# brownvc/matryodshka

Measured on AMD Instinct MI355X. Metric: novel-view frames/sec, 640x320 ODS->32-sphere MSI infer+render, higher is better.
Workload: dtype f32

## Files before the change

### matryodshka_amd/csrc/cnn_device.h

```cpp
#pragma once
#include <cmath>
#include <cstdint>
#include <cstdio>
#include <cstdlib>
#include <cstring>
#include <new>
#include <type_traits>
#include <vector>

#include "msi_common.h"

namespace msi_cnn {


typedef float f32x16 __attribute__((ext_vector_type(16)));
typedef float v4f __attribute__((ext_vector_type(4)));
typedef __attribute__((address_space(3))) void lds_void;

constexpr int BK = 32;
constexpr int ROW_BYTES = BK * 4;
#ifndef MSI_NSTAGE
#define MSI_NSTAGE 2
#endif
constexpr int NSTAGE = MSI_NSTAGE;
constexpr int NPAD_ALIGN = 128;
constexpr int COORD_CLASSES = 5;
[[maybe_unused]] constexpr unsigned OOB = 0x80000000u;
constexpr int DEFAULT_CUS = 256;
constexpr int MAX_SPLIT = 8;
constexpr int CONV_SLOTS_PER_CU = 5;
constexpr double LN_EPS = 1e-12;
constexpr int LN_SHARDS = 64, LN_WORDS = 2;
constexpr int LN_S1_BITS = 24, LN_S2_BITS = 16;
constexpr int LN_SCL_DOUBLES = 4;
constexpr double LN_UNDERFLOW_UNITS_SQ = 1e12;
enum { STATUS_APPLY_AHEAD_TIMEOUT = 1, STATUS_LN_OVERFLOW = 2, STATUS_LN_UNDERFLOW = 4, STATUS_F16_SPLIT_RANGE = 8 };
constexpr int AP_FLAG_STRIDE = 16;
constexpr int HEAD_MAX_C = 256;

enum { MODE_CONV = 0, MODE_CONVT = 1, MODE_HEAD = 2 };

struct ConvParams {
  const char *x0, *x1;
  const char *wpk;
  const char *wpk_x3;
  const float *coord_bias;
  int cb_stride;
  const double *ln_scl;
  const double *ln_scl_src, *ln_scl_src1;
  int *status;
  const long long *ln_sums;
  const float *ln_gamma, *ln_beta;
  double ln_inv_n;
  const long long *ln_sums1;
  const float *ln_gamma1, *ln_beta1;
  double ln_inv_n1;
  int halo_apply;
  const float *bias;
  float *y;
  long long *sums;
  float *partial;
  int *tile_cnt;
  int tiles_m, tiles_n, ntiles;
  int n_main, split0, split;
  int nb_main;
  int C0, C1;
  int Hin, Win, Hout, Wout, Cout, npad;
  int Mh, Mw;
  unsigned mg_mw, mg_tm, mg_tn, mg_nc, mg_sp0, mg_sp;
  int ntaps, cpt0, cpt1, ksteps;
  int stride, rate, pad_t, pad_l;
  int mode, wrap, nclass;
  int halo_tx;
  unsigned mg_htx;
  int halo_xor;
  int row_par;
  float *ap_x;
  unsigned short *ap_yb;
  const long long *ap_sums;
  const float *ap_gamma, *ap_beta;
  float *ap_aff;
  int *ap_flags;
  int *ap_err;
  double ap_inv_n;
  int n_apply, ap_units_per_row, ap_unit_vec, ap_row_vec;
#if defined(MSI_CONV_TIMING) || defined(MSI_DEBUG_STATS)
  unsigned long long *dbg;
#endif
};

enum ConvFamily {
  CONV_IGEMM = 0,
  CONV_HALO, CONV_HALO_S2, CONVT_HALO,
  CONV_HALO_X3, CONV_HALO8_X3, CONV_HALO_S2_X3, CONV_HALO8_S2_X3, CONVT_HALO_X3, CONVT_HALO8_X3,
  CONV_HALO_BF16, CONV_HALO_BF16_S2, CONVT_HALO_BF16,
};
struct ConvVariant {
  int family;
  int bm, bn;
  int mode, bf16;
  int rate;
  int apply;
  int planes;
  int waves;
  bool is_halo() const { return family != CONV_IGEMM; }
  bool is_convt_f32() const { return family == CONVT_HALO || family == CONVT_HALO_X3 || family == CONVT_HALO8_X3; }
  bool is_convt() const { return is_convt_f32() || family == CONVT_HALO_BF16; }
  bool six_product() const { return family >= CONV_HALO_X3 && family <= CONVT_HALO8_X3; }
  bool tile8() const { return family == CONV_HALO8_X3 || family == CONV_HALO8_S2_X3 || family == CONVT_HALO8_X3; }
};

struct LayerLaunch {
  ConvParams p;
  ConvVariant variant;
  int nblocks, nfix;
  int inlaunch;
  int fuse_ln;
  int skip_apply;
  unsigned ln_blocks;
};

constexpr int HA_TP = 32;
#ifndef MSI_HA_LG
#define MSI_HA_LG 32
#endif
constexpr int HA_LG = MSI_HA_LG;

struct HeadAsmParams {
  const float *x;
  const float *wpk;
  const float *bias;
  const float *aff;
  const void *psv;
  float4 *rgba;
  float *bw_out, *al_out;
  float *pred_out;
  int C0, ksteps, npad, nd, hw;
  int lg, ng;
  unsigned mg_vpp, mg_nchunk, mg_hw;
  long npix_total;
  void *layers;
};

int launch_conv(const LayerLaunch &Q, const ConvParams &p, hipStream_t stream);
int launch_igemm(const LayerLaunch &Q, const ConvParams &p, hipStream_t stream);
int launch_fixup(int bm, int bn, int mode, int raw16, unsigned grid_x, unsigned grid_y, const ConvParams &p, hipStream_t stream);
int launch_halo_f32(const LayerLaunch &Q, const ConvParams &p, hipStream_t stream);
int launch_x3(const LayerLaunch &Q, const ConvParams &p, hipStream_t stream);
int launch_bf16_halo(const LayerLaunch &Q, const ConvParams &p, hipStream_t stream);
int launch_zero(void *p, size_t n16, hipStream_t stream);
int launch_ln_finish(int batch, hipStream_t stream, const long long *sums, double inv_n, const double *scl, int *status, const float *gamma, const float *beta, int C,
                     float *aff, int raw16);
int launch_ln_apply(int bf16out, unsigned blocks, int batch, size_t lds, hipStream_t stream, float *x, const long long *sums, double inv_n, const double *scl, int *status,
                    const float *gamma, const float *beta, size_t per_sample, int C, float *aff, unsigned short *yb);
int launch_head_assemble(int bf16in, int format, unsigned grid_x, size_t lds, hipStream_t stream, const HeadAsmParams &q);
int debug_conv_occupancy(int lds_bytes);

constexpr int vkey(int family, int a = 0, int b = 0, int c = 0, int d = 0, int e = 0) { return ((((family * 16 + a) * 16 + b) * 16 + c) * 16 + d) * 16 + e; }

inline int set_max_lds(const void *fn, int lds, unsigned long long &done, const char *what) {
  int dev = 0;
  if (hipGetDevice(&dev) != hipSuccess) dev = 0;
  const bool tracked = dev >= 0 && dev < 64;
  if (tracked && ((done >> dev) & 1ull)) return MSI_OK;
  hipError_t e = hipFuncSetAttribute(fn, hipFuncAttributeMaxDynamicSharedMemorySize, lds);
  if (e != hipSuccess) return msi::fail(MSI_E_LAUNCH, "%s: %s", what, hipGetErrorString(e));
  if (tracked) done |= 1ull << dev;
  return MSI_OK;
}

template <auto KERNEL, int LDS, int THREADS = 256>
int launch_kernel(unsigned nblocks, const ConvParams &p, hipStream_t stream, const char *what) {
  if constexpr (LDS > 65536) {
    static thread_local unsigned long long done = 0;
    int rc0 = set_max_lds(reinterpret_cast<const void *>(KERNEL), LDS, done, what);
    if (rc0) return rc0;
  }
  hipLaunchKernelGGL(KERNEL, dim3(nblocks), dim3(THREADS), LDS, stream, p);
  return msi::check_launch(what);
}

template <int N> using IC = std::integral_constant<int, N>;
}
using namespace msi_cnn;

namespace {

template <int MODE>
__device__ __forceinline__ int tap_delta(int v, int parity, int rate, bool wrapt) {
  if (MODE == MODE_CONV) return v * rate;
  if (MODE == MODE_CONVT) return wrapt ? -v : (v == 0 ? 0 : (parity ? 1 : -1));
  return 0;
}

__device__ __forceinline__ unsigned udiv_magic(unsigned x, unsigned d, unsigned mg) {
  unsigned q = __umulhi(x, mg);
  if (x - q * d >= d) ++q;
  return q;
}

__device__ __forceinline__ int halo_row(const ConvParams &p, int tyi, int r, int rows_per_tile) {
  return p.row_par ? (tyi >> 1) * (2 * rows_per_tile) + (tyi & 1) + 2 * r : tyi * rows_per_tile + r;
}

__device__ __forceinline__ float msi_tanh(float x) {
  const float xa = fminf(fabsf(x), 15.0f);
  const float t = __builtin_amdgcn_exp2f(xa * 2.8853900817779268f);
  const float r = (t - 1.0f) * __builtin_amdgcn_rcpf(t + 1.0f);
  return x != x ? x : __builtin_copysignf(r, x);
}

__device__ __forceinline__ int coord_class(int mw, int Mw) {
  return mw < 2 ? mw : (mw >= Mw - 2 ? 3 + (mw - (Mw - 2)) : 2);
}

template <int N>
__device__ __forceinline__ void wait_vmcnt() {
  asm volatile("s_waitcnt vmcnt(%0)" ::"n"(N) : "memory");
}

template <int OFF>
__device__ __forceinline__ v4f lds_read128(unsigned addr) {
  v4f v;
  if constexpr (OFF < 65536) {
    asm volatile("ds_read_b128 %0, %1 offset:%2" : "=v"(v) : "v"(addr), "n"(OFF) : "memory");
  } else {
    asm volatile("ds_read_b128 %0, %1 offset:%2" : "=v"(v) : "v"(addr + (OFF & ~0xffff)), "n"(OFF & 0xffff) : "memory");
  }
  return v;
}
template <int N>
__device__ __forceinline__ void wait_lgkm(v4f &x, v4f &y) {
  asm volatile("s_waitcnt lgkmcnt(%2)" : "+v"(x), "+v"(y) : "n"(N) : "memory");
}
template <int N, int MT, int NT>
__device__ __forceinline__ void wait_lgkm_frag(v4f (&a)[MT], v4f (&b)[NT]) {
  static_assert((MT == 1 || MT == 2 || MT == 4) && (NT == 1 || NT == 2), "fragment shapes of the conv kernels");
  if constexpr (MT == 1 && NT == 1) asm volatile("s_waitcnt lgkmcnt(%2)" : "+v"(a[0]), "+v"(b[0]) : "n"(N) : "memory");
  else if constexpr (MT == 2 && NT == 1) asm volatile("s_waitcnt lgkmcnt(%3)" : "+v"(a[0]), "+v"(a[1]), "+v"(b[0]) : "n"(N) : "memory");
  else if constexpr (MT == 1 && NT == 2) asm volatile("s_waitcnt lgkmcnt(%3)" : "+v"(a[0]), "+v"(b[0]), "+v"(b[1]) : "n"(N) : "memory");
  else if constexpr (MT == 2 && NT == 2) asm volatile("s_waitcnt lgkmcnt(%4)" : "+v"(a[0]), "+v"(a[1]), "+v"(b[0]), "+v"(b[1]) : "n"(N) : "memory");
  else if constexpr (MT == 4 && NT == 1) asm volatile("s_waitcnt lgkmcnt(%5)" : "+v"(a[0]), "+v"(a[1]), "+v"(a[2]), "+v"(a[3]), "+v"(b[0]) : "n"(N) : "memory");
  else asm volatile("s_waitcnt lgkmcnt(%6)" : "+v"(a[0]), "+v"(a[1]), "+v"(a[2]), "+v"(a[3]), "+v"(b[0]), "+v"(b[1]) : "n"(N) : "memory");
}

__device__ __forceinline__ float wave_sum(float x) {
#define MSI_DPP_ADD(CTRL, ROWMASK)                                                                                     \
  x += __builtin_bit_cast(float, __builtin_amdgcn_update_dpp(0, __builtin_bit_cast(int, x), CTRL, ROWMASK, 0xf, true))
  MSI_DPP_ADD(0xB1, 0xf);
  MSI_DPP_ADD(0x4E, 0xf);
  MSI_DPP_ADD(0x141, 0xf);
  MSI_DPP_ADD(0x140, 0xf);
  MSI_DPP_ADD(0x142, 0xa);
  MSI_DPP_ADD(0x143, 0xc);
#undef MSI_DPP_ADD
  return __builtin_bit_cast(float, __builtin_amdgcn_readlane(__builtin_bit_cast(int, x), 63));
}

__device__ __forceinline__ double wave_sum_f64(double x) {
#define MSI_DPP_ADD64(CTRL, ROWMASK)                                                                                   \
  {                                                                                                                    \
    const long long b_ = __builtin_bit_cast(long long, x);                                                             \
    const int lo_ = __builtin_amdgcn_update_dpp(0, (int)b_, CTRL, ROWMASK, 0xf, true);                                 \
    const int hi_ = __builtin_amdgcn_update_dpp(0, (int)(b_ >> 32), CTRL, ROWMASK, 0xf, true);                         \
    x += __builtin_bit_cast(double, ((long long)hi_ << 32) | (unsigned)lo_);                                           \
  }
  MSI_DPP_ADD64(0xB1, 0xf) MSI_DPP_ADD64(0x4E, 0xf) MSI_DPP_ADD64(0x141, 0xf) MSI_DPP_ADD64(0x140, 0xf)
  MSI_DPP_ADD64(0x142, 0xa) MSI_DPP_ADD64(0x143, 0xc)
#undef MSI_DPP_ADD64
  const long long b = __builtin_bit_cast(long long, x);
  const int lo = __builtin_amdgcn_readlane((int)b, 63), hi = __builtin_amdgcn_readlane((int)(b >> 32), 63);
  return __builtin_bit_cast(double, ((long long)hi << 32) | (unsigned)lo);
}

__device__ __forceinline__ void ln_atomic_add(long long *dst, double x_scaled, int *status) {
  const double MAGIC = 6755399441055744.0;
  if (!(fabs(x_scaled) < 2251799813685248.0 )) {
    if (status) __hip_atomic_fetch_or(status, STATUS_LN_OVERFLOW, __ATOMIC_RELAXED, __HIP_MEMORY_SCOPE_AGENT);
    return;
  }
  const double t = x_scaled + MAGIC;
  const long long v = __builtin_bit_cast(long long, t) - __builtin_bit_cast(long long, MAGIC);
  __hip_atomic_fetch_add(dst, v, __ATOMIC_RELAXED, __HIP_MEMORY_SCOPE_AGENT);
}

struct LnShard { long long w0, w1; };
__device__ __forceinline__ LnShard ln_shard_load(const long long *sums, int tid) {
  LnShard r = {0, 0};
  if (tid < 64) {
    const long long *s = sums + (size_t)tid * LN_WORDS;
    r.w0 = s[0]; r.w1 = s[1];
  }
  return r;
}
template <bool PRE>
__device__ __forceinline__ void ln_mean_inv_impl(const long long *sums, LnShard pre, double inv_n, const double *scl, int *status, double *s_stat, int tid) {
  static_assert(LN_SHARDS == 64, "one shard per lane of wave 0");
  const double inv_s1 = scl[2], inv_s2 = scl[3];
  if (tid < 64) {
    long long w0 = pre.w0, w1 = pre.w1;
    if constexpr (!PRE) {
      const long long *s = sums + (size_t)tid * LN_WORDS;
      w0 = s[0]; w1 = s[1];
    }
    const double h1 = wave_sum_f64((double)w0), h2 = wave_sum_f64((double)w1);
    if (tid == 0) {
      const double S1 = h1 * inv_s1, S2 = h2 * inv_s2;
      if (status && h2 * h2 < LN_UNDERFLOW_UNITS_SQ * (1.0 / (inv_n * 1024.0) + 1.0))
        __hip_atomic_fetch_or(status, STATUS_LN_UNDERFLOW, __ATOMIC_RELAXED, __HIP_MEMORY_SCOPE_AGENT);
      const double mu = S1 * inv_n;
      double var = S2 * inv_n - mu * mu;
      var = var > 0.0 ? var : 0.0;
      const double x = var + LN_EPS, hx = 0.5 * x;
      double r = __builtin_amdgcn_rsq(x);
      r = r * (1.5 - hx * r * r);
      r = r * (1.5 - hx * r * r);
      s_stat[0] = mu;
      s_stat[1] = r;
    }
  }
  __syncthreads();
}
__device__ __forceinline__ void ln_mean_inv(const long long *sums, double inv_n, const double *scl, int *status, double *s_stat, int tid) {
  ln_mean_inv_impl<false>(sums, LnShard{0, 0}, inv_n, scl, status, s_stat, tid);
}
__device__ __forceinline__ void ln_mean_inv_pre(LnShard pre, double inv_n, const double *scl, int *status, double *s_stat, int tid) {
  ln_mean_inv_impl<true>(nullptr, pre, inv_n, scl, status, s_stat, tid);
}

typedef unsigned u32x4_t __attribute__((ext_vector_type(4)));

#ifndef MSI_HANDOFF_FENCE
#define MSI_HANDOFF_FENCE 0
#endif
#ifndef MSI_HANDOFF_AUX
#define MSI_HANDOFF_AUX 16
#endif
__device__ __forceinline__ void handoff_release() {
  if (MSI_HANDOFF_FENCE & 1) __builtin_amdgcn_fence(__ATOMIC_RELEASE, "agent");
}
__device__ __forceinline__ void handoff_acquire() {
  if (MSI_HANDOFF_FENCE & 2) __builtin_amdgcn_fence(__ATOMIC_ACQUIRE, "agent");
}

template <int MT, int NT, int AUX>
__device__ __forceinline__ void dump_acc(const f32x16 (&acc)[MT][NT], __amdgpu_buffer_rsrc_t rsrc, int tid) {
#pragma unroll
  for (int i = 0; i < MT; ++i)
#pragma unroll
    for (int j = 0; j < NT; ++j)
#pragma unroll
      for (int g = 0; g < 4; ++g) {
        const v4f v = {acc[i][j][4 * g], acc[i][j][4 * g + 1], acc[i][j][4 * g + 2], acc[i][j][4 * g + 3]};
        __builtin_amdgcn_raw_buffer_store_b128(__builtin_bit_cast(u32x4_t, v), rsrc,
                                               (unsigned)((((i * NT + j) * 4 + g) * 256 + tid) * 16), 0, AUX);
      }
}

template <int MT, int NT, int AUX>
__device__ __forceinline__ void sum_slabs(f32x16 (&acc)[MT][NT], __amdgpu_buffer_rsrc_t rsrc, int nsp, int slab_bytes, int tid) {
  for (int s = 0; s < nsp; ++s) {
    v4f t[MT][NT][4];
#pragma unroll
    for (int i = 0; i < MT; ++i)
#pragma unroll
      for (int j = 0; j < NT; ++j)
#pragma unroll
        for (int g = 0; g < 4; ++g)
          t[i][j][g] = __builtin_bit_cast(v4f, (u32x4_t)__builtin_amdgcn_raw_buffer_load_b128(
              rsrc, (unsigned)((((i * NT + j) * 4 + g) * 256 + tid) * 16), s * slab_bytes, AUX));
#pragma unroll
    for (int i = 0; i < MT; ++i)
#pragma unroll
      for (int j = 0; j < NT; ++j)
#pragma unroll
        for (int g = 0; g < 4; ++g) {
          if (s == 0) {
            acc[i][j][4 * g] = t[i][j][g].x; acc[i][j][4 * g + 1] = t[i][j][g].y;
            acc[i][j][4 * g + 2] = t[i][j][g].z; acc[i][j][4 * g + 3] = t[i][j][g].w;
          } else {
            acc[i][j][4 * g] += t[i][j][g].x; acc[i][j][4 * g + 1] += t[i][j][g].y;
            acc[i][j][4 * g + 2] += t[i][j][g].z; acc[i][j][4 * g + 3] += t[i][j][g].w;
          }
        }
  }
}

constexpr int EPI_STAGE_BYTES = 48 * 1024;
#ifndef MSI_EPI_NT
#define MSI_EPI_NT 0
#endif
#ifndef MSI_EPI_ABLATE
#define MSI_EPI_ABLATE 0
#endif
#ifdef MSI_CONV_TIMING
#define MSI_STAMP(k) { if (p.dbg && tid == 0) p.dbg[(size_t)blockIdx.x * 24 + (k)] = __builtin_amdgcn_s_memtime(); }
#else
#define MSI_STAMP(k)
#endif
template <int BM, int BN, int MODE, int RAW16, bool CB, bool STAGED, int WR>
__device__ __forceinline__ void emit_whole_tile(const ConvParams &p, f32x16 (&acc)[BM / (32 * WR)][BN / 64], int tile_m, int tile_n, int cls,
                                                int b, int tid, const v4f (&cb_pre)[4], bool use_pre, float pivot, float raw_mul,
                                                double scl_s1, double scl_s2, char *stage) {
  constexpr int MT = BM / (32 * WR), NT = BN / 64, NG = NT * 4, YSZ = RAW16 ? 2 : 4;
  constexpr int ROWB = NT * 32 * YSZ, PITCH = ROWB + 16, NP = ROWB / 16, PPI = 64 / NP, NRD = 32 / PPI;
  constexpr bool FITS = 2 * WR * MT * 32 * PITCH <= EPI_STAGE_BYTES;
  typedef float v2f __attribute__((ext_vector_type(2)));
  typedef _Float16 h2_t __attribute__((ext_vector_type(2)));
  typedef unsigned u2_t __attribute__((ext_vector_type(2)));
  const int lane = tid & 63, wave = tid >> 6, wm = wave >> 1, wn = wave & 1, half = lane >> 5;
  const int ph = cls >> 1, pw = cls & 1;
  const int mtot = p.Mh * p.Mw;
  const bool want_stats = p.sums != nullptr;
  const float pv_s = pivot * raw_mul;
  const v2f rm = {raw_mul, raw_mul}, pv = {pv_s, pv_s};
  const int nbw = tile_n * BN + wn * (NT * 32), nb0 = nbw + 4 * half;
  const size_t sample_bytes = (size_t)(MODE == MODE_CONVT ? p.Hout * p.Wout : mtot) * p.Cout * YSZ;
  constexpr bool staged = STAGED;
  static_assert(!STAGED || FITS, "staging strips");
  const int tyi = p.halo_tx ? (int)udiv_magic((unsigned)tile_m, (unsigned)p.halo_tx, p.mg_htx) : 0;
  const int txi = tile_m - tyi * p.halo_tx;
  MSI_STAMP(16)
  char *yp[MT];
  const float *cbp[MT];
#pragma unroll
  for (int i = 0; i < MT; ++i) {
    yp[i] = nullptr; cbp[i] = nullptr;
    if (CB || !staged) {
      int m = tile_m * BM + wm * (MT * 32) + i * 32 + (lane & 31);
      if (p.halo_tx) {
        const int local = wm * (MT * 32) + i * 32 + (lane & 31);
        m = halo_row(p, tyi, local >> 4, BM / 16) * p.Mw + txi * 16 + ((local & 15) ^ (((local >> 4) & 1) * p.halo_xor));
      }
      int mh = 0, mw = 0;
      if (MODE == MODE_CONVT || CB) {
        mh = (int)udiv_magic((unsigned)m, (unsigned)p.Mw, p.mg_mw);
        mw = m - mh * p.Mw;
      }
      const size_t opix = MODE == MODE_CONVT ? ((size_t)b * p.Hout + (2 * mh + ph)) * p.Wout + (2 * mw + pw) : (size_t)b * mtot + m;
      yp[i] = reinterpret_cast<char *>(p.y) + (opix * p.Cout + nb0) * YSZ;
      if (CB) cbp[i] = p.coord_bias + (size_t)(mh * COORD_CLASSES + coord_class(mw, p.Mw)) * p.cb_stride + nb0;
    }
  }
  char *wst = stage + wave * (MT * 32 * PITCH);
  const int slot = p.halo_tx ? ((lane & 16) | ((lane & 15) ^ (((lane >> 4) & 1) * p.halo_xor))) : (lane & 31);
  char *wp = wst + slot * PITCH + half * (4 * YSZ);
  v2f s1v[4] = {}, s2v[4] = {};
#pragma unroll
  for (int i = 0; i < MT; ++i) {
    v2f ya[NG], yc[NG];
#pragma unroll
    for (int q = 0; q < NG; ++q) {
      ya[q] = v2f{acc[i][q >> 2][4 * (q & 3)], acc[i][q >> 2][4 * (q & 3) + 1]};
      yc[q] = v2f{acc[i][q >> 2][4 * (q & 3) + 2], acc[i][q >> 2][4 * (q & 3) + 3]};
    }
    if (CB) {
      v4f cb[NG];
#pragma unroll
      for (int q = 0; q < NG; ++q)
        cb[q] = (MT == 1 && NT == 1 && use_pre) ? cb_pre[q & 3] : *reinterpret_cast<const v4f *>(cbp[i] + (q >> 2) * 32 + 8 * (q & 3));
#pragma unroll
      for (int q = 0; q < NG; ++q) { ya[q] += v2f{cb[q].x, cb[q].y}; yc[q] += v2f{cb[q].z, cb[q].w}; }
    }
    if (RAW16) {
#pragma unroll
      for (int q = 0; q < NG; ++q) { ya[q] *= rm; yc[q] *= rm; }
    }
    u2_t hw[NG];
    if (RAW16) {
#pragma unroll
      for (int q = 0; q < NG; ++q) {
        const h2_t lo = {(_Float16)ya[q].x, (_Float16)ya[q].y}, hi = {(_Float16)yc[q].x, (_Float16)yc[q].y};
        hw[q] = u2_t{__builtin_bit_cast(unsigned, lo), __builtin_bit_cast(unsigned, hi)};
      }
    }
    if (!(MSI_EPI_ABLATE & 1)) {
#pragma unroll
      for (int q = 0; q < NG; ++q) {
        char *dst = staged ? wp + i * (32 * PITCH) : yp[i];
        if (RAW16) *reinterpret_cast<u2_t *>(dst + ((q >> 2) * 32 + 8 * (q & 3)) * 2) = hw[q];
        else *reinterpret_cast<v4f *>(dst + ((q >> 2) * 32 + 8 * (q & 3)) * 4) = v4f{ya[q].x, ya[q].y, yc[q].x, yc[q].y};
      }
    }
    if (want_stats && !(MSI_EPI_ABLATE & 4)) {
#pragma unroll
      for (int q = 0; q < NG; ++q) { ya[q] -= pv; yc[q] -= pv; }
#pragma unroll
      for (int q = 0; q < NG; ++q) { s1v[q & 3] += ya[q]; s1v[q & 3] += yc[q]; }
#pragma unroll
      for (int q = 0; q < NG; ++q) {
        s2v[q & 3] = __builtin_elementwise_fma(ya[q], ya[q], s2v[q & 3]);
        s2v[q & 3] = __builtin_elementwise_fma(yc[q], yc[q], s2v[q & 3]);
      }
    }
  }
  MSI_STAMP(21)
  const v2f t1 = (s1v[0] + s1v[1]) + (s1v[2] + s1v[3]), t2 = (s2v[0] + s2v[1]) + (s2v[2] + s2v[3]);
  float s1 = t1.x + t1.y, s2 = t2.x + t2.y;
  if (staged && !(MSI_EPI_ABLATE & 1)) {
    const char *rp = wst + (lane / NP) * PITCH + (lane % NP) * 16;
    v4f pc[MT][NRD];
#pragma unroll
    for (int i = 0; i < MT; ++i)
#pragma unroll
      for (int k = 0; k < NRD; ++k) pc[i][k] = *reinterpret_cast<const v4f *>(rp + (i * 32 + k * PPI) * PITCH);
    const __amdgpu_buffer_rsrc_t rsrc_y = __builtin_amdgcn_make_buffer_rsrc(reinterpret_cast<char *>(p.y) + (size_t)b * sample_bytes, 0, (int)(unsigned)sample_bytes, 0x00020000);
    const int rowb = p.Cout * YSZ;
    int pix0, rowstep, colstep;
    if (p.halo_tx) {
      const int r0 = halo_row(p, tyi, wm * (MT * 2), BM / 16), c0 = txi * 16 + lane / NP;
      if (MODE == MODE_CONVT) { pix0 = (2 * r0 + ph) * p.Wout + 2 * c0 + pw; rowstep = 2 * p.Wout; colstep = 2; }
      else { pix0 = r0 * p.Mw + c0; rowstep = p.row_par ? 2 * p.Mw : p.Mw; colstep = 1; }
    } else {
      pix0 = tile_m * BM + wm * (MT * 32) + lane / NP; rowstep = 16; colstep = 1;
    }
    const unsigned v0 = (unsigned)pix0 * (unsigned)rowb + (unsigned)(nbw * YSZ + (lane % NP) * 16);
#pragma unroll
    for (int i = 0; i < MT; ++i)
#pragma unroll
      for (int k = 0; k < NRD; ++k) {
        const int ro = 2 * i + ((k * PPI) >> 4), co = (k * PPI) & 15;
        __builtin_amdgcn_raw_buffer_store_b128(__builtin_bit_cast(u32x4_t, pc[i][k]), rsrc_y, v0 + (unsigned)((ro * rowstep + co * colstep) * rowb), 0, MSI_EPI_NT ? 2 : 0);
      }
  }
  MSI_STAMP(17)
  if (want_stats) {
    s1 = wave_sum(s1); s2 = wave_sum(s2);
    MSI_STAMP(18)
    if (lane == 0 && !(MSI_EPI_ABLATE & 2)) {
      const double P = (double)pv_s, n = (double)(MT * NT * 16 * 64), a = (double)s1;
      const double u1 = RAW16 ? 16777216.0 : scl_s1, u2 = RAW16 ? 65536.0 : scl_s2;
      if (RAW16 && !(s2 <= 1.0727e9f)) __hip_atomic_fetch_or(p.status, STATUS_LN_OVERFLOW, __ATOMIC_RELAXED, __HIP_MEMORY_SCOPE_AGENT);
      long long *dst = p.sums + ((size_t)b * LN_SHARDS + ((blockIdx.x * 4 + wave) & (LN_SHARDS - 1))) * LN_WORDS;
      ln_atomic_add(dst, (n * P + a) * u1, p.status);
      ln_atomic_add(dst + 1, ((double)s2 + 2.0 * P * a + n * P * P) * u2, p.status);
    }
    MSI_STAMP(19)
  }
}

template <int BM, int BN, int MODE, bool INTERIOR, int RAW16, int WR>
__device__ __forceinline__ void emit_tile_impl(const ConvParams &p, f32x16 (&acc)[BM / (32 * WR)][BN / 64], int tile_m,
                                               int tile_n, int cls, int b, int tid, const v4f (&cb_pre)[4], bool use_pre, char *stage,
                                               float raw_mul_pre) {
  constexpr int MT = BM / (32 * WR), NT = BN / 64;
  const int lane = tid & 63, wave = tid >> 6, wm = wave >> 1, wn = wave & 1, half = lane >> 5;
  const int ph = cls >> 1, pw = cls & 1;
  const int mtot = p.Mh * p.Mw;
  const bool wrapt = MODE == MODE_CONVT && p.wrap != 0;
  const bool vec_ok = (p.Cout & 3) == 0;
  const bool has_cb = MODE == MODE_CONV && p.coord_bias != nullptr;
  const bool want_stats = MODE != MODE_HEAD && p.sums != nullptr;
  const float pivot = __builtin_bit_cast(float, __builtin_amdgcn_readfirstlane(__builtin_bit_cast(int, acc[0][0][0])));
  double scl_s1 = 0.0, scl_s2 = 0.0;
  const bool have_pre = INTERIOR && RAW16 && MODE != MODE_HEAD && raw_mul_pre > 0.f;
  if ((want_stats || RAW16) && !have_pre) { scl_s1 = p.ln_scl[0]; scl_s2 = p.ln_scl[1]; }
  const float raw_mul = have_pre ? raw_mul_pre : RAW16 ? (float)(scl_s1 * (1.0 / 16777216.0)) : 1.f;
  constexpr int YSZ = RAW16 ? 2 : 4;
  float s1 = 0.f, s2 = 0.f, cnt = 0.f;
  if constexpr (INTERIOR && MODE != MODE_HEAD) {
    constexpr bool FITS = 2 * WR * MT * 32 * (NT * 32 * (RAW16 ? 2 : 4) + 16) <= EPI_STAGE_BYTES;
    const size_t sample_bytes = (size_t)(MODE == MODE_CONVT ? p.Hout * p.Wout : p.Mh * p.Mw) * p.Cout * (RAW16 ? 2 : 4);
    const bool staged = FITS && stage != nullptr && sample_bytes < 0xfffffff0ull && (p.halo_tx != 0 || MODE == MODE_CONV);
    if constexpr (FITS) {
      if (staged) {
        if (has_cb) emit_whole_tile<BM, BN, MODE, RAW16, true, true, WR>(p, acc, tile_m, tile_n, cls, b, tid, cb_pre, use_pre, pivot, raw_mul, scl_s1, scl_s2, stage);
        else emit_whole_tile<BM, BN, MODE, RAW16, false, true, WR>(p, acc, tile_m, tile_n, cls, b, tid, cb_pre, use_pre, pivot, raw_mul, scl_s1, scl_s2, stage);
        return;
      }
    }
    if (has_cb) emit_whole_tile<BM, BN, MODE, RAW16, true, false, WR>(p, acc, tile_m, tile_n, cls, b, tid, cb_pre, use_pre, pivot, raw_mul, scl_s1, scl_s2, stage);
    else emit_whole_tile<BM, BN, MODE, RAW16, false, false, WR>(p, acc, tile_m, tile_n, cls, b, tid, cb_pre, use_pre, pivot, raw_mul, scl_s1, scl_s2, stage);
    return;
  }
#pragma unroll
  for (int i = 0; i < MT; ++i) {
    int m = tile_m * BM + wm * (MT * 32) + i * 32 + (lane & 31);
    if ((MODE == MODE_CONV || MODE == MODE_CONVT) && p.halo_tx) {
      const int local = wm * (MT * 32) + i * 32 + (lane & 31);
      const int tyi = (int)udiv_magic((unsigned)tile_m, (unsigned)p.halo_tx, p.mg_htx);
      m = halo_row(p, tyi, local >> 4, BM / 16) * p.Mw + (tile_m - tyi * p.halo_tx) * 16 + ((local & 15) ^ (((local >> 4) & 1) * p.halo_xor));
      if (!INTERIOR && (tile_m - tyi * p.halo_tx) * 16 + ((local & 15) ^ (((local >> 4) & 1) * p.halo_xor)) >= p.Mw) m = mtot;
    }
    const bool mok = INTERIOR || m < mtot;
    int mh = 0, mw = 0;
    if (MODE == MODE_CONVT || has_cb) {
      mh = (int)udiv_magic((unsigned)m, (unsigned)p.Mw, p.mg_mw);
      mw = m - mh * p.Mw;
    }
    size_t opix;
    bool sok = mok;
    if (MODE == MODE_CONVT) {
      int orow = 2 * mh + ph, ocol = 2 * mw + pw;
      if (wrapt) {
        orow -= 1; ocol -= 5;
        sok = mok && orow >= 0 && orow < p.Hout && ocol >= 0 && ocol < p.Wout;
      }
      opix = ((size_t)b * p.Hout + orow) * p.Wout + ocol;
    } else {
      opix = (size_t)b * mtot + m;
    }
    const float *cbrow = has_cb ? p.coord_bias + (size_t)(mh * COORD_CLASSES + coord_class(mw, p.Mw)) * p.cb_stride : nullptr;
    char *yrow = reinterpret_cast<char *>(p.y) + opix * p.Cout * YSZ;
#pragma unroll
    for (int j = 0; j < NT; ++j) {
      const int nb = tile_n * BN + wn * (NT * 32) + j * 32 + 4 * half;
#pragma unroll
      for (int g = 0; g < 4; ++g) {
        const int n = nb + 8 * g;
        const bool ok = mok && (INTERIOR || n < p.Cout);
        v4f v = {acc[i][j][4 * g], acc[i][j][4 * g + 1], acc[i][j][4 * g + 2], acc[i][j][4 * g + 3]};
        if (ok) {
          if (has_cb) {
            const v4f cb = (MT == 1 && NT == 1 && use_pre) ? cb_pre[g] : *reinterpret_cast<const v4f *>(cbrow + n);
            v.x += cb.x; v.y += cb.y; v.z += cb.z; v.w += cb.w;
          }
          if (MODE == MODE_HEAD) {
            const v4f bs = *reinterpret_cast<const v4f *>(p.bias + n);
            v.x = msi_tanh(v.x + bs.x); v.y = msi_tanh(v.y + bs.y); v.z = msi_tanh(v.z + bs.z); v.w = msi_tanh(v.w + bs.w);
          }
          if (MSI_EPI_ABLATE & 1) {
          } else if (sok && RAW16) {
            typedef _Float16 h2_t __attribute__((ext_vector_type(2)));
            typedef unsigned u2_t __attribute__((ext_vector_type(2)));
            const h2_t lo = {(_Float16)(v.x * raw_mul), (_Float16)(v.y * raw_mul)}, hi = {(_Float16)(v.z * raw_mul), (_Float16)(v.w * raw_mul)};
            *reinterpret_cast<u2_t *>(yrow + n * 2) = u2_t{__builtin_bit_cast(unsigned, lo), __builtin_bit_cast(unsigned, hi)};
          } else if (sok) {
            float *dst = reinterpret_cast<float *>(yrow) + n;
            if (vec_ok) {
              *reinterpret_cast<v4f *>(dst) = v;
            } else {
              dst[0] = v.x;
              if (n + 1 < p.Cout) dst[1] = v.y;
              if (n + 2 < p.Cout) dst[2] = v.z;
              if (n + 3 < p.Cout) dst[3] = v.w;
            }
          }
          if (want_stats && !(MSI_EPI_ABLATE & 4)) {
            const float dx = v.x - pivot, dy = v.y - pivot, dz = v.z - pivot, dw = v.w - pivot;
            if (INTERIOR || n + 3 < p.Cout) {
              s1 += (dx + dy) + (dz + dw);
              s2 += (dx * dx + dy * dy) + (dz * dz + dw * dw);
              cnt += 4.f;
            } else {
              s1 += dx; s2 += dx * dx; cnt += 1.f;
              if (n + 1 < p.Cout) { s1 += dy; s2 += dy * dy; cnt += 1.f; }
              if (n + 2 < p.Cout) { s1 += dz; s2 += dz * dz; cnt += 1.f; }
            }
          }
        }
      }
    }
  }
  if (want_stats) {
    s1 = wave_sum(s1);
    s2 = wave_sum(s2);
    const float wcnt = INTERIOR ? (float)(MT * NT * 16 * 64) : wave_sum(cnt);
    if (lane == 0 && wcnt > 0.f && !(MSI_EPI_ABLATE & 2)) {
      const double P = (double)pivot, n = (double)wcnt, a = (double)s1;
      long long *dst = p.sums + ((size_t)b * LN_SHARDS + ((blockIdx.x * 4 + wave) & (LN_SHARDS - 1))) * LN_WORDS;
      if (RAW16 && !(s2 * raw_mul * raw_mul <= 1.0727e9f)) __hip_atomic_fetch_or(p.status, STATUS_LN_OVERFLOW, __ATOMIC_RELAXED, __HIP_MEMORY_SCOPE_AGENT);
      ln_atomic_add(dst, (n * P + a) * scl_s1, p.status);
      ln_atomic_add(dst + 1, ((double)s2 + 2.0 * P * a + n * P * P) * scl_s2, p.status);
#if defined(MSI_DEBUG_STATS)
      if (p.dbg) {
        unsigned long long *o = p.dbg + 16384 * 24 + ((size_t)((blockIdx.x + gridDim.x * blockIdx.y) * 2 + (cls & 1)) * 4 + wave) * 4;
        o[0] = ((unsigned long long)__builtin_bit_cast(unsigned, s2) << 32) | __builtin_bit_cast(unsigned, s1);
        o[1] = ((unsigned long long)__builtin_bit_cast(unsigned, pivot) << 32) | __builtin_bit_cast(unsigned, wcnt);
        o[2] = __builtin_bit_cast(unsigned long long, (n * P + a) * scl_s1);
        o[3] = __builtin_bit_cast(unsigned long long, ((double)s2 + 2.0 * P * a + n * P * P) * scl_s2);
      }
#endif
    }
  }
}

template <int BM, int BN, int MODE, int RAW16 = 0, int WR = 2>
__device__ __forceinline__ void emit_tile(const ConvParams &p, f32x16 (&acc)[BM / (32 * WR)][BN / 64], int tile_m, int tile_n,
                                          int cls, int b, int tid, const v4f (&cb_pre)[4], bool use_pre, char *stage = nullptr,
                                          float raw_mul_pre = 0.f) {
  const bool interior = !(MODE == MODE_CONVT && p.wrap != 0) && (tile_m + 1) * BM <= p.Mh * p.Mw &&
                        (tile_n + 1) * BN <= p.Cout && (p.Cout & 3) == 0;
  if (interior) emit_tile_impl<BM, BN, MODE, true, RAW16, WR>(p, acc, tile_m, tile_n, cls, b, tid, cb_pre, use_pre, stage, raw_mul_pre);
  else emit_tile_impl<BM, BN, MODE, false, RAW16, WR>(p, acc, tile_m, tile_n, cls, b, tid, cb_pre, use_pre, nullptr, 0.f);
}
template <int BM, int BN, int MODE, int RAW16 = 0, int WR = 2>
__device__ __forceinline__ void emit_tile(const ConvParams &p, f32x16 (&acc)[BM / (32 * WR)][BN / 64], int tile_m, int tile_n,
                                          int cls, int b, int tid, char *stage = nullptr, float raw_mul_pre = 0.f) {
  const v4f none[4] = {};
  emit_tile<BM, BN, MODE, RAW16, WR>(p, acc, tile_m, tile_n, cls, b, tid, none, false, stage, raw_mul_pre);
}

__device__ __forceinline__ void load_coord_bias(const ConvParams &p, int tile_m, int tile_n, int tid, v4f (&cbv)[4]) {
#pragma unroll
  for (int g = 0; g < 4; ++g) cbv[g] = v4f{0.f, 0.f, 0.f, 0.f};
  if (p.coord_bias == nullptr) return;
  const int lane = tid & 63, wave = tid >> 6, wm = wave >> 1, wn = wave & 1, half = lane >> 5;
  int m = tile_m * 64 + wm * 32 + (lane & 31);
  if (p.halo_tx) {
    const int local = wm * 32 + (lane & 31);
    const int tyi = (int)udiv_magic((unsigned)tile_m, (unsigned)p.halo_tx, p.mg_htx);
    m = halo_row(p, tyi, local >> 4, 4) * p.Mw + (tile_m - tyi * p.halo_tx) * 16 + ((local & 15) ^ (((local >> 4) & 1) * p.halo_xor));
  }
  m = min(m, p.Mh * p.Mw - 1);
  const int mh = (int)udiv_magic((unsigned)m, (unsigned)p.Mw, p.mg_mw), mw = m - mh * p.Mw;
  const float *cbrow = p.coord_bias + (size_t)(mh * COORD_CLASSES + coord_class(mw, p.Mw)) * p.cb_stride;
#pragma unroll
  for (int g = 0; g < 4; ++g) {
    const int n = min(tile_n * 64 + wn * 32 + 4 * half + 8 * g, p.cb_stride - 4);
    cbv[g] = *reinterpret_cast<const v4f *>(cbrow + n);
  }
}


#ifdef MSI_EXPERIMENTS
__device__ __forceinline__ void apply_ahead(const ConvParams &p, char *smem, int tid) {
  float *s_aff = reinterpret_cast<float *>(smem);
  double *s_stat = reinterpret_cast<double *>(smem + 2 * 512 * 4 + 64);
  const int C = p.C0;
  const int upr = p.ap_units_per_row;
  const long units_per_sample = (long)p.Hin * upr;
  const int batch = p.ntiles / (p.tiles_m * p.tiles_n * p.nclass);
  const long total = units_per_sample * batch;
  const long per = (total + 7) / 8;
  const int x = blockIdx.x & 7;
  const __amdgpu_buffer_rsrc_t rs_aff = __builtin_amdgcn_make_buffer_rsrc((void *)p.ap_aff, 0, 0x7fffffff, 0x00020000);
  (void)rs_aff;
  int cur_b = -1;
  for (long l = blockIdx.x >> 3; l < per; l += p.n_apply >> 3) {
    const long u = (long)x * per + l;
    if (u >= total) break;
    const int b = (int)(u / units_per_sample);
    const long ur = u - (long)b * units_per_sample;
    const int row = (int)(ur / upr), part = (int)(ur - (long)row * upr);
    if (b != cur_b) {
      __syncthreads();
      ln_mean_inv(p.ap_sums + (size_t)b * LN_SHARDS * LN_WORDS, p.ap_inv_n, p.ln_scl_src, p.status, s_stat, tid);
      const double mu = s_stat[0], inv = s_stat[1];
      for (int c = tid; c < C; c += 256) {
        const double sc = inv * (double)p.ap_gamma[c];
        const float fs = (float)sc, ft = (float)((double)p.ap_beta[c] - mu * sc);
        s_aff[c] = fs;
        s_aff[C + c] = ft;
        if (row == 0 && part == 0) {
          p.ap_aff[(size_t)b * 2 * C + c] = fs;
          p.ap_aff[(size_t)b * 2 * C + C + c] = ft;
        }
      }
      __syncthreads();
      cur_b = b;
    }
    const size_t row_elems = (size_t)p.ap_row_vec * 4;
    const size_t base = ((size_t)b * p.Hin + row) * row_elems;
    const int v0 = part * p.ap_unit_vec;
    const int v1 = min(v0 + p.ap_unit_vec, p.ap_row_vec);
    const __amdgpu_buffer_rsrc_t rs = __builtin_amdgcn_make_buffer_rsrc((void *)(p.ap_x + base), 0, (int)(row_elems * 4), 0x00020000);
    const __amdgpu_buffer_rsrc_t rd = p.ap_yb ? __builtin_amdgcn_make_buffer_rsrc((void *)(p.ap_yb + base), 0, (int)(row_elems * 2), 0x00020000) : rs;
    auto bf16_bits = [](float f) __attribute__((always_inline)) -> unsigned {
      const unsigned uu = __builtin_bit_cast(unsigned, f);
      return (uu + 0x7fffu + ((uu >> 16) & 1u)) >> 16;
    };
    for (int v = v0 + tid; v < v1; v += 4 * 256) {
      v4f xv[4];
#pragma unroll
      for (int k = 0; k < 4; ++k)
        xv[k] = __builtin_bit_cast(v4f, (u32x4_t)__builtin_amdgcn_raw_buffer_load_b128(rs, (unsigned)((v + 256 * k) * 16), 0, 16));
#pragma unroll
      for (int k = 0; k < 4; ++k) {
        const int vv = v + 256 * k;
        if (vv >= v1) break;
        const int c = (vv * 4) % C;
        const v4f s4 = *reinterpret_cast<const v4f *>(s_aff + c), t4 = *reinterpret_cast<const v4f *>(s_aff + C + c);
        v4f y;
        y.x = fmaxf(xv[k].x * s4.x + t4.x, 0.f); y.y = fmaxf(xv[k].y * s4.y + t4.y, 0.f);
        y.z = fmaxf(xv[k].z * s4.z + t4.z, 0.f); y.w = fmaxf(xv[k].w * s4.w + t4.w, 0.f);
        if (p.ap_yb) {
          typedef unsigned v2u_t __attribute__((ext_vector_type(2)));
          const v2u_t o = {bf16_bits(y.x) | (bf16_bits(y.y) << 16), bf16_bits(y.z) | (bf16_bits(y.w) << 16)};
          __builtin_amdgcn_raw_buffer_store_b64(o, rd, (unsigned)(vv * 8), 0, 16);
        } else {
          __builtin_amdgcn_raw_buffer_store_b128(__builtin_bit_cast(u32x4_t, y), rs, (unsigned)(vv * 16), 0, 16);
        }
      }
    }
    asm volatile("s_waitcnt vmcnt(0)" ::: "memory");
    __syncthreads();
    if (tid == 0) __hip_atomic_fetch_add(p.ap_flags + ((size_t)b * p.Hin + row) * AP_FLAG_STRIDE, 1, __ATOMIC_RELAXED, __HIP_MEMORY_SCOPE_AGENT);
  }
}

__device__ __forceinline__ int rows_probe(const ConvParams &p, int b, int r0, int r1, int tid) {
  const int r = r0 + tid;
  if (r > r1) return 0x7fffffff;
  return __hip_atomic_load(p.ap_flags + ((size_t)b * p.Hin + r) * AP_FLAG_STRIDE, __ATOMIC_RELAXED, __HIP_MEMORY_SCOPE_AGENT);
}

__device__ __forceinline__ void rows_wait(const ConvParams &p, int b, int r0, int r1, int probed, int tid, int *s_flag) {
  const bool ready = probed >= p.ap_units_per_row;
  if (tid < 64) {
    const bool all = __builtin_amdgcn_ballot_w64(!ready) == 0;
    if (tid == 0) *s_flag = all ? 1 : 0;
  }
  __syncthreads();
  if (*s_flag) return;
  if (tid == 0) {
    int spins = 0;
    for (int r = r1; r >= r0; --r) {
      const int *f = p.ap_flags + ((size_t)b * p.Hin + r) * AP_FLAG_STRIDE;
      while (__hip_atomic_load(f, __ATOMIC_RELAXED, __HIP_MEMORY_SCOPE_AGENT) < p.ap_units_per_row) {
        __builtin_amdgcn_s_sleep(32);
        if (++spins > (1 << 20)) { __hip_atomic_fetch_or(p.ap_err, STATUS_APPLY_AHEAD_TIMEOUT, __ATOMIC_RELAXED, __HIP_MEMORY_SCOPE_AGENT); r = r0; break; }
      }
    }
  }
  __syncthreads();
}

#endif

__device__ constexpr int s2_tap(int J) { return J == 0 ? 0 : J == 1 ? 2 : J == 2 ? 6 : J == 3 ? 8 : J == 4 ? 1 : J == 5 ? 7 : J == 6 ? 3 : J == 7 ? 5 : 4; }
__device__ constexpr int s2_unit(int J) { return J < 4 ? 0 : J < 6 ? 1 : J < 8 ? 2 : 3; }

}
```

### matryodshka_amd/csrc/cnn_igemm.hip

```cpp
#include "cnn_device.h"

namespace {

template <int BM, int BN, int MODE, int BF16>
__global__ void __launch_bounds__(256) __attribute__((amdgpu_waves_per_eu(BM * BN >= 128 * 128 ? 2 : (BM * BN > 64 * 64 || NSTAGE > 2 ? 3 : 5))))
conv_igemm_kernel(const ConvParams p) {
#if defined(__HIP_DEVICE_COMPILE__)
  constexpr int ESZ = BF16 ? 2 : 4;
  constexpr int BKE = ROW_BYTES / ESZ;
  constexpr int MT = BM / 64, NT = BN / 64;
  constexpr int AI = BM / 32, BI = BN / 32;
  constexpr int STAGE_BYTES = (BM + BN) * ROW_BYTES;
  extern __shared__ __attribute__((aligned(16))) char smem[];

#ifdef MSI_CONV_TIMING
  const unsigned long long ts0 = __builtin_amdgcn_s_memtime(), ts0r = __builtin_amdgcn_s_memrealtime();
#endif
  const int tid = threadIdx.x, lane = tid & 63;
  const int wave = __builtin_amdgcn_readfirstlane(tid >> 6);
  const int wm = wave >> 1, wn = wave & 1;
#ifdef MSI_EXPERIMENTS
  if (p.n_apply > 0 && (int)blockIdx.x < p.n_apply) {
    apply_ahead(p, smem, tid);
    return;
  }
#endif
  const int S = p.ksteps;
  int t, k0 = 0, k1 = S, ks = 0, slot = 0;
  {
#ifdef MSI_EXPERIMENTS
    const int bid = (int)blockIdx.x - p.n_apply;
#else
    const int bid = (int)blockIdx.x;
#endif
    if (bid < p.nb_main && p.split0 == 1) {
      const int q = p.n_main >> 3, r = p.n_main & 7, xcd = bid & 7, local = bid >> 3;
      t = (xcd < r ? xcd * (q + 1) : r * (q + 1) + (xcd - r) * q) + local;
    } else {
      int sp, r, tbase;
      unsigned mg;
      if (bid < p.nb_main) { sp = p.split0; mg = p.mg_sp0; r = bid; tbase = 0; }
      else { sp = p.split; mg = p.mg_sp; r = bid - p.nb_main; tbase = p.n_main; }
      const int tl = (int)udiv_magic((unsigned)r, (unsigned)sp, mg);
      ks = r - tl * sp;
      t = tbase + tl;
      k0 = (int)udiv_magic((unsigned)(ks * S), (unsigned)sp, mg);
      k1 = (int)udiv_magic((unsigned)((ks + 1) * S), (unsigned)sp, mg);
      slot = bid - (p.split0 == 1 ? p.nb_main : 0);
    }
  }
  const bool full = (k0 == 0) & (k1 == S);
  int tile_m, tile_n, cls, b;
  {
    int r = t;
    const int q0 = (int)udiv_magic((unsigned)r, (unsigned)p.nclass, p.mg_nc);
    cls = r - q0 * p.nclass; r = q0;
    const int q1 = (int)udiv_magic((unsigned)r, (unsigned)p.tiles_m, p.mg_tm);
    tile_m = r - q1 * p.tiles_m; r = q1;
    const int q2 = (int)udiv_magic((unsigned)r, (unsigned)p.tiles_n, p.mg_tn);
    tile_n = r - q2 * p.tiles_n;
    b = q2;
  }
  constexpr bool CB_PRE = BM == 64 && BN == 64 && MODE == MODE_CONV && !BF16;
  v4f cbv[4];
  if constexpr (CB_PRE) load_coord_bias(p, tile_m, tile_n, tid, cbv);
  const int ph = cls >> 1, pw = cls & 1;
  const int mtot = p.Mh * p.Mw;
  const int wrap_w = p.wrap ? p.Win : 0;
  const bool wrapt = MODE == MODE_CONVT && p.wrap != 0;
#ifdef MSI_EXPERIMENTS
  int ap_r0 = 0, ap_r1 = -1, ap_probe = 0;
  if (p.n_apply > 0) {
    const int m_lo = tile_m * BM, m_hi = min(m_lo + BM, mtot) - 1;
    const int mh_lo = (int)udiv_magic((unsigned)m_lo, (unsigned)p.Mw, p.mg_mw), mh_hi = (int)udiv_magic((unsigned)m_hi, (unsigned)p.Mw, p.mg_mw);
    if (MODE == MODE_CONV) { ap_r0 = mh_lo * p.stride - p.pad_t; ap_r1 = mh_hi * p.stride - p.pad_t + 2 * p.rate; }
    else if (MODE == MODE_CONVT) { ap_r0 = mh_lo - 1; ap_r1 = wrapt ? mh_hi : mh_hi + 1; }
    else { ap_r0 = mh_lo; ap_r1 = mh_hi; }
    ap_r0 = max(ap_r0, 0);
    ap_r1 = min(ap_r1, p.Hin - 1);
    ap_probe = rows_probe(p, b, ap_r0, ap_r1, tid);
  }
#endif

  const int drow = lane >> 3, dslot = lane & 7;
  constexpr int NV = MODE == MODE_CONV ? 3 : (MODE == MODE_CONVT ? 2 : 1);
  int rowbase[AI], colw0[AI], colw1[AI], colw2[AI];
  unsigned vmask[AI], a_chunk16[AI];
#pragma unroll
  for (int i = 0; i < AI; ++i) {
    const int r = wave * (BM / 4) + i * 8 + drow;
    const int m = tile_m * BM + r;
    const int mh = (int)udiv_magic((unsigned)m, (unsigned)p.Mw, p.mg_mw);
    const int mw = m - mh * p.Mw;
    const int ih0 = mh * p.stride - p.pad_t, iw0 = mw * p.stride - p.pad_l;
    rowbase[i] = ih0 * p.Win;
    const bool mok = m < mtot;
    unsigned rowok = 0, colok = 0;
    colw1[i] = colw2[i] = 0;
#pragma unroll
    for (int v = 0; v < NV; ++v) {
      const int ih = ih0 + tap_delta<MODE>(v, ph, p.rate, wrapt);
      const int iwu = iw0 + tap_delta<MODE>(v, pw, p.rate, wrapt);
      const int iw = iwu < 0 ? iwu + wrap_w : (iwu >= p.Win ? iwu - wrap_w : iwu);
      if (v == 0) colw0[i] = iw;
      if (v == 1) colw1[i] = iw;
      if (v == 2) colw2[i] = iw;
      if (ih >= 0 && ih < p.Hin) rowok |= 1u << v;
      if (iw >= 0 && iw < p.Win && !(wrapt && (iwu < -2 || iwu >= p.Win + 2))) colok |= 1u << v;
    }
    unsigned colrep = 0, rowrep = 0;
#pragma unroll
    for (int vr = 0; vr < NV; ++vr) {
      colrep |= colok << (vr * NV);
      rowrep |= ((rowok >> vr) & 1u) * (((1u << NV) - 1u) << (vr * NV));
    }
    const unsigned vm = mok ? (colrep & rowrep) : 0u;
    vmask[i] = vm;
    a_chunk16[i] = (unsigned)((dslot ^ ((r >> 1) & 7)) * 16);
  }
  const unsigned b_voff = (unsigned)((tile_n * BN + wave * (BN / 4) + drow) * ROW_BYTES + dslot * 16);

  const size_t in_pix = (size_t)p.Hin * p.Win;
  const __amdgpu_buffer_rsrc_t rsrc_b = __builtin_amdgcn_make_buffer_rsrc(
      (void *)(p.wpk + (size_t)cls * S * p.npad * ROW_BYTES), 0, (int)((size_t)S * p.npad * ROW_BYTES), 0x00020000);
  const char *src0 = p.x0 + (size_t)b * in_pix * p.C0 * ESZ;
  const long d_src = (p.x1 + (size_t)b * in_pix * p.C1 * ESZ) - src0;
  const int bytes0 = (int)(in_pix * p.C0 * ESZ), bytes1 = (int)(in_pix * p.C1 * ESZ);

  unsigned a_voff[AI];
  __amdgpu_buffer_rsrc_t rsrc_a = __builtin_amdgcn_make_buffer_rsrc((void *)src0, 0, bytes0, 0x00020000);
  const int nreg = p.ntaps * (p.cpt0 + p.cpt1);
  int g_step = k0, g_tap = 0, g_src = 0, g_chunk = 0, g_C = p.C0;
  if (k0 > 0 && k0 < nreg) {
    const int cpt = p.cpt0 + p.cpt1;
    g_tap = k0 / cpt;
    const int within = k0 - g_tap * cpt;
    g_src = within >= p.cpt0 ? 1 : 0;
    g_chunk = g_src ? within - p.cpt0 : within;
  }

  bool g_new = true;
#define MSI_ISSUE(stage)                                                                                  \
  {                                                                                                                              \
                                     \
    char *sA = smem + (stage) * STAGE_BYTES + wave * (BM / 4) * ROW_BYTES;                                                         \
    char *sB = smem + (stage) * STAGE_BYTES + BM * ROW_BYTES + wave * (BN / 4) * ROW_BYTES;                                        \
    const int soff_b = g_step * p.npad * ROW_BYTES;                                                                              \
           \
           \
                                            \
    static_assert(BI <= 4, "B rows per wave: written out for immediate offsets");                                                \
    __builtin_amdgcn_raw_ptr_buffer_load_lds(rsrc_b, (lds_void *)sB, 16, b_voff, soff_b, 0, 0);                                  \
    if (BI > 1) __builtin_amdgcn_raw_ptr_buffer_load_lds(rsrc_b, (lds_void *)sB, 16, b_voff, soff_b, 8 * ROW_BYTES, 0);          \
    if (BI > 2) __builtin_amdgcn_raw_ptr_buffer_load_lds(rsrc_b, (lds_void *)sB, 16, b_voff, soff_b, 16 * ROW_BYTES, 0);         \
    if (BI > 3) __builtin_amdgcn_raw_ptr_buffer_load_lds(rsrc_b, (lds_void *)sB, 16, b_voff, soff_b, 24 * ROW_BYTES, 0);         \
    if (g_step < nreg) {                                                                                                         \
      if (g_new) {                                                                                                               \
                                          \
        g_new = false;                                                                                                           \
        int vr, vc;                                                                                                              \
        if (MODE == MODE_CONV) { vr = g_tap / 3; vc = g_tap - vr * 3; }                                                          \
        else if (MODE == MODE_CONVT) { vr = g_tap >> 1; vc = g_tap & 1; }                                                        \
        else { vr = 0; vc = 0; }                                                                                                 \
        const int srow = tap_delta<MODE>(vr, ph, p.rate, wrapt) * p.Win;                                                         \
        const unsigned bit = 1u << (vr * NV + vc);                                                                               \
        g_C = g_src ? p.C1 : p.C0;                                                                                               \
        rsrc_a = __builtin_amdgcn_make_buffer_rsrc((void *)(src0 + (g_src ? d_src : 0L)), 0, g_src ? bytes1 : bytes0,            \
                                                   0x00020000);                                                                  \
        const unsigned pix_bytes = (unsigned)g_C * (unsigned)ESZ;                                                                           \
_Pragma("unroll")                                                                                                                \
        for (int i = 0; i < AI; ++i) {                                                                                           \
          int iw = colw0[i];                                                                                                     \
          if (NV > 1) iw = vc == 1 ? colw1[i] : iw;                                                                              \
          if (NV > 2) iw = vc == 2 ? colw2[i] : iw;                                                                              \
                                \
                                                                                     \
          const unsigned off = __umul24((unsigned)(rowbase[i] + srow + iw), pix_bytes) + a_chunk16[i];                           \
          a_voff[i] = (vmask[i] & bit) != 0 ? off : OOB;                                                                         \
        }                                                                                                                        \
      }                                                                                                                          \
      const int soff_a = g_chunk * ROW_BYTES;                                                                                    \
      const int cleft = g_C - g_chunk * BKE;         \
      if (MODE == MODE_HEAD && !BF16 && p.ln_sums != nullptr) {                                                                  \
              \
              \
        const float *aff_ = s_haff;                                                                                              \
_Pragma("unroll")                                                                                                                \
        for (int i = 0; i < AI; ++i) {                                                                                           \
          typedef unsigned u32x4 __attribute__((ext_vector_type(4)));                                                            \
          const v4f x = __builtin_bit_cast(v4f, (u32x4)__builtin_amdgcn_raw_buffer_load_b128(rsrc_a, a_voff[i], soff_a, 0)); \
          const int c0 = g_chunk * BKE + (int)(a_chunk16[i] >> 2);                                                               \
          const v4f s4 = *reinterpret_cast<const v4f *>(aff_ + c0), t4 = *reinterpret_cast<const v4f *>(aff_ + p.C0 + c0);       \
          v4f y;                                                                                                                 \
          y.x = fmaxf(x.x * s4.x + t4.x, 0.f); y.y = fmaxf(x.y * s4.y + t4.y, 0.f);                                              \
          y.z = fmaxf(x.z * s4.z + t4.z, 0.f); y.w = fmaxf(x.w * s4.w + t4.w, 0.f);                                              \
          *reinterpret_cast<v4f *>(sA + i * 8 * ROW_BYTES + lane * 16) = y;                                                      \
        }                                                                                                                        \
      } else if (cleft >= BKE) {                                                                                                 \
_Pragma("unroll")                                                                                                                \
        for (int i = 0; i < AI; ++i)                                                                                             \
          __builtin_amdgcn_raw_ptr_buffer_load_lds(rsrc_a, (lds_void *)(sA + i * 8 * ROW_BYTES), 16, a_voff[i], soff_a, 0, 0);   \
      } else {                                                                                                                   \
                                    \
_Pragma("unroll")                                                                                                                \
        for (int i = 0; i < AI; ++i)                                                                                             \
          __builtin_amdgcn_raw_ptr_buffer_load_lds(rsrc_a, (lds_void *)(sA + i * 8 * ROW_BYTES), 16,                             \
                                                   a_chunk16[i] < (unsigned)(cleft * ESZ) ? a_voff[i] : OOB, soff_a, 0, 0);         \
      }                                                                                                                          \
    }                                                                                                                            \
                                                                                        \
    ++g_step;                                                                                                                    \
    if (g_step < nreg) {                                                                                                         \
      ++g_chunk;                                                                                                                 \
      const int cpt = g_src ? p.cpt1 : p.cpt0;                                                                                   \
      if (g_chunk == cpt) {                                                                                                      \
        g_chunk = 0;                                                                                                             \
        if (g_src == 0 && p.cpt1 > 0) {                                                                                          \
          g_src = 1;                                                                                                             \
        } else {                                                                                                                 \
          g_src = 0;                                                                                                             \
          ++g_tap;                                                                                                               \
        }                                                                                                                        \
        g_new = true;                                                                                                            \
      }                                                                                                                          \
    }                                                                                                                            \
  }

#ifdef MSI_EXPERIMENTS
  if (p.n_apply > 0) rows_wait(p, b, ap_r0, ap_r1, ap_probe, tid, reinterpret_cast<int *>(smem));
#endif

  float *s_haff = nullptr;
  if constexpr (MODE == MODE_HEAD && !BF16) {
    __shared__ __attribute__((aligned(16))) float s_haff_store[2 * HEAD_MAX_C];
    __shared__ double s_hstat[2];
    s_haff = s_haff_store;
    if (p.ln_sums != nullptr) {
      ln_mean_inv(p.ln_sums + (size_t)b * LN_SHARDS * LN_WORDS, p.ln_inv_n, p.ln_scl_src, p.status, s_hstat, tid);
      const double mu = s_hstat[0], inv = s_hstat[1];
      for (int c = tid; c < p.C0; c += 256) {
        const double sc = inv * (double)p.ln_gamma[c];
        s_haff_store[c] = (float)sc;
        s_haff_store[p.C0 + c] = (float)((double)p.ln_beta[c] - mu * sc);
      }
      __syncthreads();
    }
  }

  const int nsteps = k1 - k0;
  MSI_ISSUE(0)

  const int frow = lane & 31, fh = lane >> 5;
  const int fswz = (frow >> 1) & 7;
  unsigned a_q[4], b_q[4];
  {
    const unsigned lds_base = (unsigned)(size_t)(lds_void *)smem;
#pragma unroll
    for (int q = 0; q < 4; ++q) {
      const int slot = ((BF16 ? 2 * q + fh : fh * 4 + q) ^ fswz) * 16;
      a_q[q] = lds_base + (wm * (MT * 32) + frow) * ROW_BYTES + slot;
      b_q[q] = lds_base + BM * ROW_BYTES + (wn * (NT * 32) + frow) * ROW_BYTES + slot;
    }
  }

  f32x16 acc[MT][NT];
#pragma unroll
  for (int i = 0; i < MT; ++i)
#pragma unroll
    for (int j = 0; j < NT; ++j)
#pragma unroll
      for (int r = 0; r < 16; ++r) acc[i][j][r] = 0.f;

  struct Frag { v4f a[4][MT], b[4][NT]; };
#define MSI_FETCH(F, ST)                                                                              \
  _Pragma("unroll") for (int q_ = 0; q_ < 4; ++q_) {                                                  \
    _Pragma("unroll") for (int i_ = 0; i_ < MT; ++i_)                                                 \
      F.a[q_][i_] = i_ == 0 ? lds_read128<(ST) * STAGE_BYTES>(a_q[q_])                                \
                            : lds_read128<(ST) * STAGE_BYTES + (MT - 1) * 32 * ROW_BYTES>(a_q[q_]);    \
    _Pragma("unroll") for (int j_ = 0; j_ < NT; ++j_)                                                 \
      F.b[q_][j_] = j_ == 0 ? lds_read128<(ST) * STAGE_BYTES>(b_q[q_])                                \
                            : lds_read128<(ST) * STAGE_BYTES + (NT - 1) * 32 * ROW_BYTES>(b_q[q_]);    \
  }
  static_assert(MT <= 2 && NT <= 2, "MSI_FETCH addresses at most two MFMA tiles per direction");
  typedef __bf16 bf16x8 __attribute__((ext_vector_type(8)));
  auto mma_quarter = [&](Frag &f, const int q) __attribute__((always_inline)) {
#pragma unroll
    for (int i = 0; i < MT; ++i)
#pragma unroll
      for (int j = 0; j < NT; ++j) {
        if constexpr (BF16) {
          acc[i][j] = __builtin_amdgcn_mfma_f32_32x32x16_bf16(__builtin_bit_cast(bf16x8, f.b[q][j]),
                                                              __builtin_bit_cast(bf16x8, f.a[q][i]), acc[i][j], 0, 0, 0);
        } else {
          acc[i][j] = __builtin_amdgcn_mfma_f32_32x32x2f32(f.b[q][j].x, f.a[q][i].x, acc[i][j], 0, 0, 0);
          acc[i][j] = __builtin_amdgcn_mfma_f32_32x32x2f32(f.b[q][j].y, f.a[q][i].y, acc[i][j], 0, 0, 0);
          acc[i][j] = __builtin_amdgcn_mfma_f32_32x32x2f32(f.b[q][j].z, f.a[q][i].z, acc[i][j], 0, 0, 0);
          acc[i][j] = __builtin_amdgcn_mfma_f32_32x32x2f32(f.b[q][j].w, f.a[q][i].w, acc[i][j], 0, 0, 0);
        }
      }
  };
#define MSI_MMA_Q(F, Q)                                                                           \
  wait_lgkm_frag<(3 - (Q)) * (MT + NT), MT, NT>(F.a[Q], F.b[Q]);                                  \
  mma_quarter(F, Q);                                                                              \
  __builtin_amdgcn_sched_barrier(0);

  static_assert(NSTAGE == 2 || NSTAGE == 3, "the main loop is unrolled for a 2- or 3-stage ring");
  constexpr int PD = NSTAGE - 1;
  constexpr int DMA_PER_STEP = AI + BI;
  if (PD > 1 && nsteps > 1) {
    MSI_ISSUE(1)
    wait_vmcnt<DMA_PER_STEP>();
  } else {
    wait_vmcnt<0>();
  }
  asm volatile("s_waitcnt lgkmcnt(0)" ::: "memory");
  __builtin_amdgcn_s_barrier();

#define MSI_KSTEP(U, S)                                                                   \
  {                                                                                       \
    Frag f_;                                                                              \
    MSI_FETCH(f_, U)                                                                      \
    MSI_MMA_Q(f_, 0)                                                                      \
    const bool more_ = (S) + PD < nsteps;                                                 \
    if (more_) MSI_ISSUE(((U) + PD) % NSTAGE)                                             \
    MSI_MMA_Q(f_, 1)                                                                      \
    MSI_MMA_Q(f_, 2)                                                                      \
    MSI_MMA_Q(f_, 3)                                                                      \
    if (PD > 1 && more_) wait_vmcnt<(PD - 1) * DMA_PER_STEP>(); else wait_vmcnt<0>();     \
    __builtin_amdgcn_s_barrier();                                                         \
  }
#ifdef MSI_CONV_TIMING
  const unsigned long long ts1 = __builtin_amdgcn_s_memtime();
#endif
  for (int S = 0; S < nsteps; S += NSTAGE) {
    MSI_KSTEP(0, S);
    if (S + 1 >= nsteps) break;
    MSI_KSTEP(1, S + 1);
    if (NSTAGE > 2) {
      if (S + 2 >= nsteps) break;
      MSI_KSTEP(NSTAGE - 1, S + 2);
    }
  }
#undef MSI_KSTEP
#ifdef MSI_CONV_TIMING
  const unsigned long long ts2 = __builtin_amdgcn_s_memtime();
  auto stamp = [&]() __attribute__((always_inline)) {
    if (p.dbg && tid == 0) {
      unsigned long long *o = p.dbg + (size_t)blockIdx.x * 24;
      o[0] = ts0; o[1] = ts1; o[2] = ts2; o[3] = __builtin_amdgcn_s_memtime(); o[22] = ts0r; o[23] = __builtin_amdgcn_s_memrealtime();
      o[4] = __builtin_amdgcn_s_getreg(4 | (31 << 11));
      o[5] = __builtin_amdgcn_s_getreg(20 | (31 << 11));
    }
  };
#endif
#undef MSI_ISSUE
#undef MSI_MMA_Q
#undef MSI_FETCH

  if (!full) {
    constexpr int SLAB = BM * BN * 4;
    const __amdgpu_buffer_rsrc_t rsrc_p = __builtin_amdgcn_make_buffer_rsrc(
        (void *)(p.partial + (size_t)slot * (BM * BN)), 0, SLAB, 0x00020000);
    if (p.tile_cnt == nullptr) {
      dump_acc<MT, NT, 0>(acc, rsrc_p, tid);
#ifdef MSI_CONV_TIMING
      stamp();
#endif
      return;
    }
    dump_acc<MT, NT, MSI_HANDOFF_AUX>(acc, rsrc_p, tid);
    const int nsp = t < p.n_main ? p.split0 : p.split;
    asm volatile("s_waitcnt vmcnt(0)" ::: "memory");
    handoff_release();
    __syncthreads();
    int *s_old = reinterpret_cast<int *>(smem);
    if (tid == 0) {
      *s_old = __hip_atomic_fetch_add(p.tile_cnt + (t - (p.split0 == 1 ? p.n_main : 0)), 1, __ATOMIC_RELAXED,
                                      __HIP_MEMORY_SCOPE_AGENT);
    }
    __syncthreads();
    if (*s_old != nsp - 1) {
#ifdef MSI_CONV_TIMING
      stamp();
#endif
      return;
    }
    handoff_acquire();
    const __amdgpu_buffer_rsrc_t rsrc_t = __builtin_amdgcn_make_buffer_rsrc(
        (void *)(p.partial + (size_t)(slot - ks) * (BM * BN)), 0, nsp * SLAB, 0x00020000);
    sum_slabs<MT, NT, MSI_HANDOFF_AUX>(acc, rsrc_t, nsp, SLAB, tid);
    __syncthreads();
  }
  static_assert((size_t)2 * (BM + BN) * ROW_BYTES >= (size_t)4 * (BM / 64) * 32 * ((BN / 64) * 32 * (BF16 ? 2 : 4) + 16), "staging strips");
  emit_tile<BM, BN, MODE, (BF16 && MODE != MODE_HEAD) ? 1 : 0>(p, acc, tile_m, tile_n, cls, b, tid, cbv, CB_PRE && p.coord_bias != nullptr, smem);
#ifdef MSI_CONV_TIMING
  stamp();
#endif
#endif
}

template <int BM, int BN, int MODE, int RAW16 = 0>
__global__ void __launch_bounds__(256)
conv_fixup_kernel(const ConvParams p) {
#if defined(__HIP_DEVICE_COMPILE__)
  constexpr int MT = BM / 64, NT = BN / 64;
  const int tid = threadIdx.x;
  const int t = (p.split0 == 1 ? p.n_main : 0) + blockIdx.x;
  const int nsp = t < p.n_main ? p.split0 : p.split;
  const int slot0 = p.split0 == 1 ? (t - p.n_main) * p.split
                                  : (t < p.n_main ? t * p.split0 : p.nb_main + (t - p.n_main) * p.split);
  int tile_m, tile_n, cls, b;
  {
    int r = t;
    const int q0 = (int)udiv_magic((unsigned)r, (unsigned)p.nclass, p.mg_nc);
    cls = r - q0 * p.nclass; r = q0;
    const int q1 = (int)udiv_magic((unsigned)r, (unsigned)p.tiles_m, p.mg_tm);
    tile_m = r - q1 * p.tiles_m; r = q1;
    const int q2 = (int)udiv_magic((unsigned)r, (unsigned)p.tiles_n, p.mg_tn);
    tile_n = r - q2 * p.tiles_n;
    b = q2;
  }
  constexpr int SLAB = BM * BN * 4;
  f32x16 acc[MT][NT];
  if (MODE == MODE_CONVT && p.halo_tx) {
    const int pwc = blockIdx.y;
    cls = 2 * cls + pwc;
    const __amdgpu_buffer_rsrc_t rsrc_h = __builtin_amdgcn_make_buffer_rsrc(
        (void *)(p.partial + ((size_t)slot0 * 2 + pwc) * (BM * BN)), 0, nsp * 2 * SLAB, 0x00020000);
    sum_slabs<MT, NT, 0>(acc, rsrc_h, nsp, 2 * SLAB, tid);
  } else {
    const __amdgpu_buffer_rsrc_t rsrc_t = __builtin_amdgcn_make_buffer_rsrc(
        (void *)(p.partial + (size_t)slot0 * (BM * BN)), 0, nsp * SLAB, 0x00020000);
    sum_slabs<MT, NT, 0>(acc, rsrc_t, nsp, SLAB, tid);
  }
  emit_tile<BM, BN, MODE, RAW16>(p, acc, tile_m, tile_n, cls, b, tid);
#endif
}

template <int BM, int BN, int MODE, int BF16>
int launch_conv_mode(const LayerLaunch &Q, const ConvParams &p, hipStream_t stream) {
  return launch_kernel<conv_igemm_kernel<BM, BN, MODE, BF16>, NSTAGE * (BM + BN) * ROW_BYTES>(Q.nblocks + p.n_apply, p, stream, "conv_igemm");
}

}

namespace msi_cnn {
int launch_igemm(const LayerLaunch &Q, const ConvParams &p, hipStream_t stream) {
  const ConvVariant &V = Q.variant;
  switch (vkey(V.family, V.bm / 64, V.bn / 64, V.mode, V.bf16)) {
    case vkey(CONV_IGEMM, 1, 1, MODE_CONV, 0): return launch_conv_mode<64, 64, MODE_CONV, 0>(Q, p, stream);
    case vkey(CONV_IGEMM, 1, 1, MODE_CONVT, 0): return launch_conv_mode<64, 64, MODE_CONVT, 0>(Q, p, stream);
    case vkey(CONV_IGEMM, 1, 1, MODE_HEAD, 0): return launch_conv_mode<64, 64, MODE_HEAD, 0>(Q, p, stream);
    case vkey(CONV_IGEMM, 1, 1, MODE_CONV, 1): return launch_conv_mode<64, 64, MODE_CONV, 1>(Q, p, stream);
    case vkey(CONV_IGEMM, 1, 1, MODE_CONVT, 1): return launch_conv_mode<64, 64, MODE_CONVT, 1>(Q, p, stream);
    case vkey(CONV_IGEMM, 1, 1, MODE_HEAD, 1): return launch_conv_mode<64, 64, MODE_HEAD, 1>(Q, p, stream);
    case vkey(CONV_IGEMM, 2, 1, MODE_CONV, 1): return launch_conv_mode<128, 64, MODE_CONV, 1>(Q, p, stream);
    case vkey(CONV_IGEMM, 2, 1, MODE_CONVT, 1): return launch_conv_mode<128, 64, MODE_CONVT, 1>(Q, p, stream);
    case vkey(CONV_IGEMM, 2, 1, MODE_HEAD, 1): return launch_conv_mode<128, 64, MODE_HEAD, 1>(Q, p, stream);
    case vkey(CONV_IGEMM, 2, 2, MODE_CONV, 1): return launch_conv_mode<128, 128, MODE_CONV, 1>(Q, p, stream);
    case vkey(CONV_IGEMM, 2, 2, MODE_CONVT, 1): return launch_conv_mode<128, 128, MODE_CONVT, 1>(Q, p, stream);
    case vkey(CONV_IGEMM, 2, 2, MODE_HEAD, 1): return launch_conv_mode<128, 128, MODE_HEAD, 1>(Q, p, stream);
#ifdef MSI_EXPERIMENTS
    case vkey(CONV_IGEMM, 2, 1, MODE_CONV, 0): return launch_conv_mode<128, 64, MODE_CONV, 0>(Q, p, stream);
    case vkey(CONV_IGEMM, 2, 1, MODE_CONVT, 0): return launch_conv_mode<128, 64, MODE_CONVT, 0>(Q, p, stream);
    case vkey(CONV_IGEMM, 1, 2, MODE_CONV, 0): return launch_conv_mode<64, 128, MODE_CONV, 0>(Q, p, stream);
    case vkey(CONV_IGEMM, 1, 2, MODE_CONVT, 0): return launch_conv_mode<64, 128, MODE_CONVT, 0>(Q, p, stream);
#endif
  }
  return msi::fail(MSI_E_UNSUPPORTED, "conv: no conv_igemm_kernel<%d, %d, %d, %d> (fp32: the 64x64 tile; 128x64 and 64x128 are experiments, MSI_EXPERIMENTS)", V.bm, V.bn, V.mode, V.bf16);
}
int launch_fixup(int bm, int bn, int mode, int raw16, unsigned gx, unsigned gy, const ConvParams &p, hipStream_t stream) {
  const dim3 grid(gx, gy), block(256);
  switch (bn == 64 ? vkey(bm / 64, mode, raw16 ? 1 : 0) : -1) {
    case vkey(1, MODE_CONV, 0): hipLaunchKernelGGL((conv_fixup_kernel<64, 64, MODE_CONV, 0>), grid, block, 0, stream, p); break;
    case vkey(1, MODE_CONVT, 0): hipLaunchKernelGGL((conv_fixup_kernel<64, 64, MODE_CONVT, 0>), grid, block, 0, stream, p); break;
    case vkey(1, MODE_HEAD, 0): hipLaunchKernelGGL((conv_fixup_kernel<64, 64, MODE_HEAD, 0>), grid, block, 0, stream, p); break;
    case vkey(1, MODE_CONV, 1): hipLaunchKernelGGL((conv_fixup_kernel<64, 64, MODE_CONV, 1>), grid, block, 0, stream, p); break;
    case vkey(1, MODE_CONVT, 1): hipLaunchKernelGGL((conv_fixup_kernel<64, 64, MODE_CONVT, 1>), grid, block, 0, stream, p); break;
    case vkey(2, MODE_CONV, 0): hipLaunchKernelGGL((conv_fixup_kernel<128, 64, MODE_CONV, 0>), grid, block, 0, stream, p); break;
    case vkey(2, MODE_CONVT, 0): hipLaunchKernelGGL((conv_fixup_kernel<128, 64, MODE_CONVT, 0>), grid, block, 0, stream, p); break;
    default: return msi::fail(MSI_E_UNSUPPORTED, "conv_fixup: tile %d x %d, mode %d%s", bm, bn, mode, raw16 ? ", fp16 raw output" : "");
  }
  return msi::check_launch("conv_fixup");
}
int debug_conv_occupancy(int lds_bytes) {
  int n = -1;
  (void)hipOccupancyMaxActiveBlocksPerMultiprocessor(&n, conv_igemm_kernel<64, 64, MODE_CONV, 0>, 256, (size_t)lds_bytes);
  return n;
}
}
```

### matryodshka_amd/csrc/cnn_x3.hip

```cpp
#include "cnn_device.h"

namespace {

#ifndef MSI_X3_EARLY_DMA
#define MSI_X3_EARLY_DMA 0
#endif
#ifndef MSI_X3_NSTG
#define MSI_X3_NSTG 0
#endif
#ifndef MSI_X3_ABLATE
#define MSI_X3_ABLATE 0
#endif
#ifndef MSI_X2_NSTG
#define MSI_X2_NSTG 3
#endif
constexpr int x3_rate_y(int RATE) { return RATE == 3 ? 1 : RATE; }
constexpr int x3_rate_x(int RATE) { return RATE == 3 ? 2 : RATE; }
constexpr int x3_nstg(int RATE, int NPL) { return NPL == 2 ? MSI_X2_NSTG : (MSI_X3_NSTG ? MSI_X3_NSTG : (RATE == 2 ? 3 : 2)); }
template <int RATE, int NS = x3_nstg(RATE, 3), int NPL = 3, int TH = 4>
struct HaloGeomX3 {
  static constexpr int PW = 16 + 2 * x3_rate_x(RATE), PH = TH + 2 * x3_rate_y(RATE), NPX = PW * PH;
  static constexpr int PIX_BYTES = NPL * 64 + 16;
  static constexpr int ROW_PITCH = ((PW * PIX_BYTES + 127) / 256) * 256 + 128;
  static constexpr int A_BYTES = PH * ROW_PITCH;
  static constexpr int B_ROW = 64;
  static constexpr int B_PLANE = 64 * B_ROW, B_STAGE = NPL * B_PLANE;
  static constexpr int NSTG = NS;
  static constexpr int LDS_BYTES = A_BYTES + NSTG * B_STAGE;
  static constexpr int NLOAD = (NPX * 8 + 255) / 256;
};
__device__ __forceinline__ void f16_range_track(unsigned &amax, v4f y) {
  const float fx = y.x, fy = y.y, fz = y.z, fw = y.w;
  const unsigned a = __builtin_bit_cast(unsigned, fx) & 0x7fffffffu, b = __builtin_bit_cast(unsigned, fy) & 0x7fffffffu;
  const unsigned c = __builtin_bit_cast(unsigned, fz) & 0x7fffffffu, d = __builtin_bit_cast(unsigned, fw) & 0x7fffffffu;
  amax = max(max(amax, a), max(b, max(c, d)));
}
constexpr unsigned F16_MAX_BITS = 0x477fe000u;

template <int N>
__device__ __forceinline__ void wait_lgkm4(v4f &a, v4f &b, v4f &c, v4f &d) {
  asm volatile("s_waitcnt lgkmcnt(%4)" : "+v"(a), "+v"(b), "+v"(c), "+v"(d) : "n"(N) : "memory");
}
template <int N>
__device__ __forceinline__ void wait_lgkm6(v4f &a, v4f &b, v4f &c, v4f &d, v4f &e, v4f &f) {
  asm volatile("s_waitcnt lgkmcnt(%6)" : "+v"(a), "+v"(b), "+v"(c), "+v"(d), "+v"(e), "+v"(f) : "n"(N) : "memory");
}

#ifndef MSI_X2_WAVES
#define MSI_X2_WAVES 4
#endif
#ifndef MSI_X2_LATE_CB
#define MSI_X2_LATE_CB 1
#endif
template <int NP>
__device__ __forceinline__ void split_mfma(f32x16 &acc, f32x16 &lo, const v4f &ah, const v4f &am, const v4f &al, const v4f &bh, const v4f &bm, const v4f &bl);
template <int RATE, int APPLY, int NPL, int TH>
__device__ __forceinline__ void conv_halo_x3_body(const ConvParams &p, char *smem) {
  typedef HaloGeomX3<RATE, x3_nstg(RATE, NPL), NPL, TH> G;
  constexpr int RY = x3_rate_y(RATE), RX = x3_rate_x(RATE), PW = G::PW, NPX = G::NPX, NLOAD = G::NLOAD;
  static_assert(RATE != 3 || TH == 4, "row-parity tiles: four rows");
  constexpr int MT = TH / 4, NT = 1, BM = 16 * TH;
  static_assert(TH == 4 || (TH == 8 && NPL == 3 && RATE == 1), "the 8-row tile is built for the six-product form at rate 1");
#ifdef MSI_CONV_TIMING
  const unsigned long long ts0 = __builtin_amdgcn_s_memtime(), ts0r = __builtin_amdgcn_s_memrealtime();
#endif
  const int tid = threadIdx.x, lane = tid & 63;
  const int wave = __builtin_amdgcn_readfirstlane(tid >> 6);
  const int wm = wave >> 1, wn = wave & 1;
  const int CH = p.cpt0;
  int t, c0 = 0, c1 = CH, ks = 0, slot = 0;
  {
    const int bid = blockIdx.x;
    if (bid < p.nb_main && p.split0 == 1) {
      const int q = p.n_main >> 3, r = p.n_main & 7, xcd = bid & 7, local = bid >> 3;
      t = (xcd < r ? xcd * (q + 1) : r * (q + 1) + (xcd - r) * q) + local;
    } else {
      int sp, r, tbase;
      unsigned mg;
      if (bid < p.nb_main) { sp = p.split0; mg = p.mg_sp0; r = bid; tbase = 0; }
      else { sp = p.split; mg = p.mg_sp; r = bid - p.nb_main; tbase = p.n_main; }
      const int tl = (int)udiv_magic((unsigned)r, (unsigned)sp, mg);
      ks = r - tl * sp;
      t = tbase + tl;
      c0 = (int)udiv_magic((unsigned)(ks * CH), (unsigned)sp, mg);
      c1 = (int)udiv_magic((unsigned)((ks + 1) * CH), (unsigned)sp, mg);
      slot = bid - (p.split0 == 1 ? p.nb_main : 0);
    }
  }
  const bool full = (c0 == 0) & (c1 == CH);
  int tile_m, tile_n, b;
  {
    int r = t;
    const int q1 = (int)udiv_magic((unsigned)r, (unsigned)p.tiles_m, p.mg_tm);
    tile_m = r - q1 * p.tiles_m; r = q1;
    const int q2 = (int)udiv_magic((unsigned)r, (unsigned)p.tiles_n, p.mg_tn);
    tile_n = r - q2 * p.tiles_n;
    b = q2;
  }
  LnShard shard = {0, 0};
  if (APPLY) shard = ln_shard_load(p.ln_sums + (size_t)b * LN_SHARDS * LN_WORDS, tid);
  const int tyi = (int)udiv_magic((unsigned)tile_m, (unsigned)p.halo_tx, p.mg_htx);
  const int ow0 = (tile_m - tyi * p.halo_tx) * 16;
  const int H = p.Hin, W = p.Win, C = p.C0;
  v4f cbv[4] = {};
  if (MT == 1 && (!MSI_X2_LATE_CB || NPL != 2)) load_coord_bias(p, tile_m, tile_n, tid, cbv);
  const int S = p.ksteps;
  const int plane_bytes = p.npad * G::B_ROW;
  const __amdgpu_buffer_rsrc_t rsrc_b = __builtin_amdgcn_make_buffer_rsrc((void *)p.wpk_x3, 0, (int)((size_t)S * NPL * plane_bytes), 0x00020000);
  const unsigned b_voff = (unsigned)((tile_n * 64 + wave * 16 + (lane >> 2)) * G::B_ROW + (lane & 3) * 16);
  int c = c0, cpar = 0;
  (void)cpar;
  auto b_issue = [&](const int c, const int tap, const int st) __attribute__((always_inline)) {
    if (MSI_X3_ABLATE & 1) return;
    char *sB_ = smem + G::A_BYTES + st * G::B_STAGE + wave * 16 * G::B_ROW;
    const int soff_ = (tap * CH + c) * NPL * plane_bytes;
    __builtin_amdgcn_raw_ptr_buffer_load_lds(rsrc_b, (lds_void *)sB_, 16, b_voff, soff_, 0, 0);
    __builtin_amdgcn_raw_ptr_buffer_load_lds(rsrc_b, (lds_void *)(sB_ + G::B_PLANE), 16, b_voff, soff_ + plane_bytes, 0, 0);
    if (NPL == 3) __builtin_amdgcn_raw_ptr_buffer_load_lds(rsrc_b, (lds_void *)(sB_ + 2 * G::B_PLANE), 16, b_voff, soff_ + 2 * plane_bytes, 0, 0);
  };
  b_issue(c0, 0, 0);
  if (G::NSTG == 3) b_issue(c0, 1, 1);

  unsigned voff[NLOAD], lds_a[NLOAD];
  bool pok[NLOAD];
  const int cslot = tid & 7;
#pragma unroll
  for (int k = 0; k < NLOAD; ++k) {
    const int pp = (tid + 256 * k) >> 3;
    const int py = pp / PW, px = pp - py * PW;
    const int ih = RATE == 3 ? (tyi >> 1) * (2 * TH) + (tyi & 1) + 2 * (py - 1) : tyi * TH - RY + py;
    int iw = ow0 - RX + px;
    if (p.wrap) iw = iw < 0 ? iw + W : (iw >= W ? iw - W : iw);
    pok[k] = pp < NPX && ih >= 0 && ih < H && iw >= 0 && iw < W;
    voff[k] = pok[k] ? __umul24((unsigned)(ih * W + iw), (unsigned)(C * 4)) + (unsigned)(cslot * 16) : OOB;
    lds_a[k] = pp < NPX ? (unsigned)(py * G::ROW_PITCH + px * G::PIX_BYTES + cslot * 8) : 0xffffffffu;
  }
  const size_t in_bytes = (size_t)H * W * C * 4;
  const __amdgpu_buffer_rsrc_t rsrc_a = __builtin_amdgcn_make_buffer_rsrc((void *)(p.x0 + (size_t)b * in_bytes), 0, (int)in_bytes, 0x00020000);

  float inv_f = 1.f, mu_hi = 0.f, mu_lo = 0.f;
  bool has_pad = false;
  if (APPLY) {
    bool bad = false;
#pragma unroll
    for (int k = 0; k < NLOAD; ++k) bad |= (lds_a[k] != 0xffffffffu) && !pok[k];
    has_pad = __builtin_amdgcn_ballot_w64(bad) != 0;
  }
  v4f araw[NLOAD], g4, be4;
  unsigned amax_ = 0u;
  auto patch_load = [&](const int c) __attribute__((always_inline)) {
#pragma unroll
    for (int k_ = 0; k_ < NLOAD; ++k_)
      araw[k_] = __builtin_bit_cast(v4f, (u32x4_t)__builtin_amdgcn_raw_buffer_load_b128(rsrc_a, voff[k_], c * ROW_BYTES, 0));
    if (APPLY) {
      g4 = *reinterpret_cast<const v4f *>(p.ln_gamma + c * 32 + cslot * 4);
      be4 = *reinterpret_cast<const v4f *>(p.ln_beta + c * 32 + cslot * 4);
    }
  };
  auto patch_store = [&]() __attribute__((always_inline)) {
    v4f s4 = {1.f, 1.f, 1.f, 1.f}, t4 = {0.f, 0.f, 0.f, 0.f};
    if (APPLY) {
      s4 = inv_f * g4;
      const v4f nh = {-mu_hi, -mu_hi, -mu_hi, -mu_hi}, nl = {-mu_lo, -mu_lo, -mu_lo, -mu_lo};
      t4 = __builtin_elementwise_fma(nl, s4, __builtin_elementwise_fma(nh, s4, be4));
    }
#pragma unroll
    for (int k_ = 0; k_ < NLOAD; ++k_) {
      v4f y = araw[k_];
      if (APPLY) {
        y = __builtin_elementwise_max(__builtin_elementwise_fma(y, s4, t4), v4f{0.f, 0.f, 0.f, 0.f});
        if (has_pad && !pok[k_]) y = v4f{0.f, 0.f, 0.f, 0.f};
      }
      if (NPL == 2) {
        typedef _Float16 h2_t __attribute__((ext_vector_type(2)));
        typedef unsigned u2x_t __attribute__((ext_vector_type(2)));
        f16_range_track(amax_, y);
        const h2_t ha = {(_Float16)y.x, (_Float16)y.y}, hb = {(_Float16)y.z, (_Float16)y.w};
        const h2_t ma = {(_Float16)((y.x - (float)ha.x) * 2048.f), (_Float16)((y.y - (float)ha.y) * 2048.f)};
        const h2_t mb = {(_Float16)((y.z - (float)hb.x) * 2048.f), (_Float16)((y.w - (float)hb.y) * 2048.f)};
        if (lds_a[k_] != 0xffffffffu) {
          *reinterpret_cast<u2x_t *>(smem + lds_a[k_]) = u2x_t{__builtin_bit_cast(unsigned, ha), __builtin_bit_cast(unsigned, hb)};
          *reinterpret_cast<u2x_t *>(smem + lds_a[k_] + 64) = u2x_t{__builtin_bit_cast(unsigned, ma), __builtin_bit_cast(unsigned, mb)};
        }
      } else {
      unsigned h0, h1, m0, m1, l0, l1;
      asm("v_cvt_pk_bf16_f32 %0, %1, %2" : "=v"(h0) : "v"(y.x), "v"(y.y));
      asm("v_cvt_pk_bf16_f32 %0, %1, %2" : "=v"(h1) : "v"(y.z), "v"(y.w));
      v4f r = y - v4f{__builtin_bit_cast(float, h0 << 16), __builtin_bit_cast(float, h0 & 0xffff0000u),
                      __builtin_bit_cast(float, h1 << 16), __builtin_bit_cast(float, h1 & 0xffff0000u)};
      asm("v_cvt_pk_bf16_f32 %0, %1, %2" : "=v"(m0) : "v"(r.x), "v"(r.y));
      asm("v_cvt_pk_bf16_f32 %0, %1, %2" : "=v"(m1) : "v"(r.z), "v"(r.w));
      r = r - v4f{__builtin_bit_cast(float, m0 << 16), __builtin_bit_cast(float, m0 & 0xffff0000u),
                  __builtin_bit_cast(float, m1 << 16), __builtin_bit_cast(float, m1 & 0xffff0000u)};
      asm("v_cvt_pk_bf16_f32 %0, %1, %2" : "=v"(l0) : "v"(r.x), "v"(r.y));
      asm("v_cvt_pk_bf16_f32 %0, %1, %2" : "=v"(l1) : "v"(r.z), "v"(r.w));
      if (lds_a[k_] != 0xffffffffu) {
        typedef unsigned u2x_t __attribute__((ext_vector_type(2)));
        *reinterpret_cast<u2x_t *>(smem + lds_a[k_]) = u2x_t{h0, h1};
        *reinterpret_cast<u2x_t *>(smem + lds_a[k_] + 64) = u2x_t{m0, m1};
        *reinterpret_cast<u2x_t *>(smem + lds_a[k_] + 128) = u2x_t{l0, l1};
      }
    }
    }
  };
  const int frow = lane & 31, fh = lane >> 5, fswz = (frow >> 1) & 7;
  const unsigned lds_base = (unsigned)(size_t)(lds_void *)smem;
  const unsigned a_base = lds_base + (unsigned)((2 * MT * wm + (frow >> 4)) * G::ROW_PITCH + ((frow & 15) ^ ((frow >> 4) << 3)) * G::PIX_BYTES + fh * 16);
  unsigned b_s[2];
  (void)fswz;
#pragma unroll
  for (int s_ = 0; s_ < 2; ++s_)
    b_s[s_] = lds_base + G::A_BYTES + (wn * 32 + frow) * G::B_ROW + (((2 * s_ + fh) ^ ((frow >> 2) & 3)) << 4);
  typedef __bf16 bf16x8 __attribute__((ext_vector_type(8)));
  typedef _Float16 f16x8 __attribute__((ext_vector_type(8)));
  f32x16 acc[MT][1], acc_lo;
#pragma unroll
  for (int i = 0; i < MT; ++i)
#pragma unroll
    for (int r = 0; r < 16; ++r) acc[i][0][r] = acc_lo[r] = 0.f;

  auto htap = [&](auto TAP_c) __attribute__((always_inline)) {
    constexpr int TAP = decltype(TAP_c)::value;
    constexpr int KH_ = TAP / 3, KW_ = TAP % 3;
    const unsigned bst_ = (unsigned)(G::NSTG == 3 ? TAP % 3 : ((TAP ^ cpar) & 1)) * G::B_STAGE;
    constexpr int AOFF_ = KH_ * RY * G::ROW_PITCH + KW_ * RX * G::PIX_BYTES;
    v4f ah_[2], am_[2], al_[2], bh_[2], bm_[2], bl_[2];
    if (MSI_X3_EARLY_DMA || G::NSTG == 2) {
      constexpr int PD_ = G::NSTG - 1;
      const int stn_ = G::NSTG == 3 ? (TAP + 2) % 3 : (((TAP ^ cpar) & 1) ^ 1);
      if (TAP + PD_ < 9) { b_issue(c, TAP + PD_, stn_); }
      else if (c + 1 < c1) { b_issue(c + 1, TAP + PD_ - 9, stn_); }
    }
    if (NPL == 2) {
#pragma unroll
      for (int s_ = 0; s_ < 2; ++s_) {
        ah_[s_] = s_ == 0 ? lds_read128<AOFF_>(a_base) : lds_read128<AOFF_ + 32>(a_base);
        bh_[s_] = lds_read128<0>(b_s[s_] + bst_);
        am_[s_] = s_ == 0 ? lds_read128<AOFF_ + 64>(a_base) : lds_read128<AOFF_ + 96>(a_base);
        bm_[s_] = lds_read128<G::B_PLANE>(b_s[s_] + bst_);
      }
#pragma unroll
      for (int s_ = 0; s_ < 2; ++s_) {
        if (s_ == 0) wait_lgkm4<4>(ah_[0], bh_[0], am_[0], bm_[0]);
        else wait_lgkm4<0>(ah_[1], bh_[1], am_[1], bm_[1]);
        acc_lo = __builtin_amdgcn_mfma_f32_32x32x16_f16(__builtin_bit_cast(f16x8, bm_[s_]), __builtin_bit_cast(f16x8, ah_[s_]), acc_lo, 0, 0, 0);
        acc[0][0] = __builtin_amdgcn_mfma_f32_32x32x16_f16(__builtin_bit_cast(f16x8, bh_[s_]), __builtin_bit_cast(f16x8, ah_[s_]), acc[0][0], 0, 0, 0);
        acc_lo = __builtin_amdgcn_mfma_f32_32x32x16_f16(__builtin_bit_cast(f16x8, bh_[s_]), __builtin_bit_cast(f16x8, am_[s_]), acc_lo, 0, 0, 0);
        __builtin_amdgcn_sched_barrier(0);
        if (s_ == 0) {
          if (TAP == 0 && c + 1 < c1) patch_load(c + 1);
          if (!MSI_X3_EARLY_DMA && G::NSTG == 3) {
            if (TAP + 2 < 9) { b_issue(c, TAP + 2, (TAP + 2) % 3); }
            else if (c + 1 < c1) { b_issue(c + 1, TAP - 7, (TAP + 2) % 3); }
          }
        }
      }
    } else if constexpr (MT == 2) {
      constexpr int A1_ = AOFF_ + 2 * G::ROW_PITCH;
      v4f xh_[2][2], xm_[2][2], xl_[2][2];
      bh_[0] = lds_read128<0>(b_s[0] + bst_); bm_[0] = lds_read128<G::B_PLANE>(b_s[0] + bst_); bl_[0] = lds_read128<2 * G::B_PLANE>(b_s[0] + bst_);
      xh_[0][0] = lds_read128<AOFF_>(a_base); xm_[0][0] = lds_read128<AOFF_ + 64>(a_base); xl_[0][0] = lds_read128<AOFF_ + 128>(a_base);
      xh_[0][1] = lds_read128<A1_>(a_base); xm_[0][1] = lds_read128<A1_ + 64>(a_base); xl_[0][1] = lds_read128<A1_ + 128>(a_base);
      bh_[1] = lds_read128<0>(b_s[1] + bst_); bm_[1] = lds_read128<G::B_PLANE>(b_s[1] + bst_); bl_[1] = lds_read128<2 * G::B_PLANE>(b_s[1] + bst_);
      wait_lgkm6<6>(bh_[0], bm_[0], bl_[0], xh_[0][0], xm_[0][0], xl_[0][0]);
      split_mfma<3>(acc[0][0], acc_lo, xh_[0][0], xm_[0][0], xl_[0][0], bh_[0], bm_[0], bl_[0]);
      __builtin_amdgcn_sched_barrier(0);
      xh_[1][0] = lds_read128<AOFF_ + 32>(a_base); xm_[1][0] = lds_read128<AOFF_ + 96>(a_base); xl_[1][0] = lds_read128<AOFF_ + 160>(a_base);
      xh_[1][1] = lds_read128<A1_ + 32>(a_base); xm_[1][1] = lds_read128<A1_ + 96>(a_base); xl_[1][1] = lds_read128<A1_ + 160>(a_base);
      if (TAP == 0 && c + 1 < c1) patch_load(c + 1);
      wait_lgkm6<9>(xh_[0][1], xm_[0][1], xl_[0][1], bh_[0], bm_[0], bl_[0]);
      split_mfma<3>(acc[1][0], acc_lo, xh_[0][1], xm_[0][1], xl_[0][1], bh_[0], bm_[0], bl_[0]);
      __builtin_amdgcn_sched_barrier(0);
      wait_lgkm6<3>(bh_[1], bm_[1], bl_[1], xh_[1][0], xm_[1][0], xl_[1][0]);
      split_mfma<3>(acc[0][0], acc_lo, xh_[1][0], xm_[1][0], xl_[1][0], bh_[1], bm_[1], bl_[1]);
      __builtin_amdgcn_sched_barrier(0);
      wait_lgkm6<0>(xh_[1][1], xm_[1][1], xl_[1][1], bh_[1], bm_[1], bl_[1]);
      split_mfma<3>(acc[1][0], acc_lo, xh_[1][1], xm_[1][1], xl_[1][1], bh_[1], bm_[1], bl_[1]);
      __builtin_amdgcn_sched_barrier(0);
    } else {
    if (!(MSI_X3_ABLATE & 8))
#pragma unroll
      for (int s_ = 0; s_ < 2; ++s_) {
      ah_[s_] = s_ == 0 ? lds_read128<AOFF_>(a_base) : lds_read128<AOFF_ + 32>(a_base);
      bh_[s_] = lds_read128<0>(b_s[s_] + bst_);
      am_[s_] = s_ == 0 ? lds_read128<AOFF_ + 64>(a_base) : lds_read128<AOFF_ + 96>(a_base);
      bm_[s_] = lds_read128<G::B_PLANE>(b_s[s_] + bst_);
      al_[s_] = s_ == 0 ? lds_read128<AOFF_ + 128>(a_base) : lds_read128<AOFF_ + 160>(a_base);
      bl_[s_] = lds_read128<2 * G::B_PLANE>(b_s[s_] + bst_);
    }
#pragma unroll
      for (int s_ = 0; s_ < 2; ++s_) {
      if (s_ == 0) wait_lgkm6<6>(ah_[0], bh_[0], am_[0], bm_[0], al_[0], bl_[0]);
      else wait_lgkm6<0>(ah_[1], bh_[1], am_[1], bm_[1], al_[1], bl_[1]);
      if (!(MSI_X3_ABLATE & 16)) {
      acc[0][0] = __builtin_amdgcn_mfma_f32_32x32x16_bf16(__builtin_bit_cast(bf16x8, bm_[s_]), __builtin_bit_cast(bf16x8, am_[s_]), acc[0][0], 0, 0, 0);
      acc[0][0] = __builtin_amdgcn_mfma_f32_32x32x16_bf16(__builtin_bit_cast(bf16x8, bh_[s_]), __builtin_bit_cast(bf16x8, al_[s_]), acc[0][0], 0, 0, 0);
      acc[0][0] = __builtin_amdgcn_mfma_f32_32x32x16_bf16(__builtin_bit_cast(bf16x8, bl_[s_]), __builtin_bit_cast(bf16x8, ah_[s_]), acc[0][0], 0, 0, 0);
      acc[0][0] = __builtin_amdgcn_mfma_f32_32x32x16_bf16(__builtin_bit_cast(bf16x8, bh_[s_]), __builtin_bit_cast(bf16x8, am_[s_]), acc[0][0], 0, 0, 0);
      acc[0][0] = __builtin_amdgcn_mfma_f32_32x32x16_bf16(__builtin_bit_cast(bf16x8, bm_[s_]), __builtin_bit_cast(bf16x8, ah_[s_]), acc[0][0], 0, 0, 0);
      acc[0][0] = __builtin_amdgcn_mfma_f32_32x32x16_bf16(__builtin_bit_cast(bf16x8, bh_[s_]), __builtin_bit_cast(bf16x8, ah_[s_]), acc[0][0], 0, 0, 0);
      }
      __builtin_amdgcn_sched_barrier(0);
      if (s_ == 0) {
        if (TAP == 0 && c + 1 < c1) patch_load(c + 1);
        if (!MSI_X3_EARLY_DMA && G::NSTG == 3) {
        if (TAP + 2 < 9) { b_issue(c, TAP + 2, (TAP + 2) % 3); }
        else if (c + 1 < c1) { b_issue(c + 1, TAP - 7, (TAP + 2) % 3); }
        }
      }
    }
    }
    {
      const bool issued_ = (TAP + 2 < 9) || (c + 1 < c1);
      if (G::NSTG == 2) {
        if (TAP == 0 && c + 1 < c1) wait_vmcnt<NLOAD + (APPLY ? 2 : 0)>();
        else wait_vmcnt<0>();
      } else if (TAP == 0 && c + 1 < c1) wait_vmcnt<NPL + NLOAD + (APPLY ? 2 : 0)>();
      else if (issued_) wait_vmcnt<NPL>();
      else wait_vmcnt<0>();
    }
    if (!(MSI_X3_ABLATE & 4)) __builtin_amdgcn_s_barrier();
  };

  patch_load(c0);
  if (APPLY) {
    double *s_stat = reinterpret_cast<double *>(smem);
    ln_mean_inv_pre(shard, p.ln_inv_n, p.ln_scl_src, p.status, s_stat, tid);
    const double mu = s_stat[0];
    inv_f = (float)s_stat[1];
    mu_hi = (float)mu;
    mu_lo = (float)(mu - (double)mu_hi);
    __syncthreads();
  }
  wait_vmcnt<0>();
  patch_store();
  asm volatile("s_waitcnt lgkmcnt(0)" ::: "memory");
  __builtin_amdgcn_s_barrier();
#ifdef MSI_CONV_TIMING
  const unsigned long long ts1 = __builtin_amdgcn_s_memtime();
#endif
  for (; c < c1; ++c) {
    cpar = (c - c0) & 1;
    htap(IC<0>{}); htap(IC<1>{}); htap(IC<2>{}); htap(IC<3>{}); htap(IC<4>{}); htap(IC<5>{}); htap(IC<6>{}); htap(IC<7>{}); htap(IC<8>{});
    if (c + 1 < c1 && !(MSI_X3_ABLATE & 32)) {
      patch_store();
      asm volatile("s_waitcnt lgkmcnt(0)" ::: "memory");
      __builtin_amdgcn_s_barrier();
    }
  }
  if (MSI_X2_LATE_CB && NPL == 2) load_coord_bias(p, tile_m, tile_n, tid, cbv);
  if (NPL == 2) {
#pragma unroll
    for (int r = 0; r < 16; ++r) acc[0][0][r] = __builtin_fmaf(acc_lo[r], 1.f / 2048.f, acc[0][0][r]);
    if (__builtin_amdgcn_ballot_w64(amax_ > F16_MAX_BITS) != 0 && lane == 0) atomicOr(p.status, STATUS_F16_SPLIT_RANGE);
  }

#ifdef MSI_CONV_TIMING
  const unsigned long long ts2 = __builtin_amdgcn_s_memtime();
  auto stamp = [&]() __attribute__((always_inline)) {
    if (p.dbg && tid == 0) {
      unsigned long long *o = p.dbg + (size_t)blockIdx.x * 24;
      o[0] = ts0; o[1] = ts1; o[2] = ts2; o[3] = __builtin_amdgcn_s_memtime(); o[22] = ts0r; o[23] = __builtin_amdgcn_s_memrealtime();
      o[4] = __builtin_amdgcn_s_getreg(4 | (31 << 11));
      o[5] = __builtin_amdgcn_s_getreg(20 | (31 << 11));
    }
  };
#endif
  if (!full) {
    constexpr int SLAB = BM * 64 * 4;
    const __amdgpu_buffer_rsrc_t rsrc_p = __builtin_amdgcn_make_buffer_rsrc((void *)(p.partial + (size_t)slot * (BM * 64)), 0, SLAB, 0x00020000);
    if (p.tile_cnt == nullptr) {
      dump_acc<MT, NT, 0>(acc, rsrc_p, tid);
#ifdef MSI_CONV_TIMING
      stamp();
#endif
      return;
    }
    dump_acc<MT, NT, MSI_HANDOFF_AUX>(acc, rsrc_p, tid);
    const int nsp = t < p.n_main ? p.split0 : p.split;
    asm volatile("s_waitcnt vmcnt(0)" ::: "memory");
    handoff_release();
    __syncthreads();
    int *s_old = reinterpret_cast<int *>(smem);
    if (tid == 0)
      *s_old = __hip_atomic_fetch_add(p.tile_cnt + (t - (p.split0 == 1 ? p.n_main : 0)), 1, __ATOMIC_RELAXED, __HIP_MEMORY_SCOPE_AGENT);
    __syncthreads();
    if (*s_old != nsp - 1) return;
    handoff_acquire();
    const __amdgpu_buffer_rsrc_t rsrc_t = __builtin_amdgcn_make_buffer_rsrc((void *)(p.partial + (size_t)(slot - ks) * (BM * 64)), 0, nsp * SLAB, 0x00020000);
    sum_slabs<MT, NT, MSI_HANDOFF_AUX>(acc, rsrc_t, nsp, SLAB, tid);
    __syncthreads();
  }
  emit_tile<BM, 64, MODE_CONV>(p, acc, tile_m, tile_n, 0, b, tid, cbv, MT == 1 && p.coord_bias != nullptr, smem);
#ifdef MSI_CONV_TIMING
  stamp();
#endif
}

template <int RATE, int APPLY, int NPL>
__global__ void __launch_bounds__(256) __attribute__((amdgpu_waves_per_eu((NPL == 2 && RATE == 1) ? MSI_X2_WAVES : 2)))
conv_halo_x3_kernel(const ConvParams p) {
#if defined(__HIP_DEVICE_COMPILE__)
  extern __shared__ __attribute__((aligned(16))) char smem[];
  conv_halo_x3_body<RATE, APPLY, NPL, 4>(p, smem);
#endif
}
template <int APPLY, int NPL>
__global__ void __launch_bounds__(256) __attribute__((amdgpu_waves_per_eu(2)))
conv_halo8_x3_kernel(const ConvParams p) {
#if defined(__HIP_DEVICE_COMPILE__)
  extern __shared__ __attribute__((aligned(16))) char smem[];
  conv_halo_x3_body<1, APPLY, NPL, 8>(p, smem);
#endif
}

template <int NP>
__device__ __forceinline__ void split_store(char *smem, unsigned off, v4f y, unsigned &amax) {
  typedef unsigned u2x_t __attribute__((ext_vector_type(2)));
  if (NP == 2) {
    typedef _Float16 h2_t __attribute__((ext_vector_type(2)));
    f16_range_track(amax, y);
    const h2_t ha = {(_Float16)y.x, (_Float16)y.y}, hb = {(_Float16)y.z, (_Float16)y.w};
    const h2_t ma = {(_Float16)((y.x - (float)ha.x) * 2048.f), (_Float16)((y.y - (float)ha.y) * 2048.f)};
    const h2_t mb = {(_Float16)((y.z - (float)hb.x) * 2048.f), (_Float16)((y.w - (float)hb.y) * 2048.f)};
    if (off != 0xffffffffu) {
      *reinterpret_cast<u2x_t *>(smem + off) = u2x_t{__builtin_bit_cast(unsigned, ha), __builtin_bit_cast(unsigned, hb)};
      *reinterpret_cast<u2x_t *>(smem + off + 64) = u2x_t{__builtin_bit_cast(unsigned, ma), __builtin_bit_cast(unsigned, mb)};
    }
  } else {
    unsigned h0, h1, m0, m1, l0, l1;
    asm("v_cvt_pk_bf16_f32 %0, %1, %2" : "=v"(h0) : "v"(y.x), "v"(y.y));
    asm("v_cvt_pk_bf16_f32 %0, %1, %2" : "=v"(h1) : "v"(y.z), "v"(y.w));
    v4f r = y - v4f{__builtin_bit_cast(float, h0 << 16), __builtin_bit_cast(float, h0 & 0xffff0000u),
                    __builtin_bit_cast(float, h1 << 16), __builtin_bit_cast(float, h1 & 0xffff0000u)};
    asm("v_cvt_pk_bf16_f32 %0, %1, %2" : "=v"(m0) : "v"(r.x), "v"(r.y));
    asm("v_cvt_pk_bf16_f32 %0, %1, %2" : "=v"(m1) : "v"(r.z), "v"(r.w));
    r = r - v4f{__builtin_bit_cast(float, m0 << 16), __builtin_bit_cast(float, m0 & 0xffff0000u),
                __builtin_bit_cast(float, m1 << 16), __builtin_bit_cast(float, m1 & 0xffff0000u)};
    asm("v_cvt_pk_bf16_f32 %0, %1, %2" : "=v"(l0) : "v"(r.x), "v"(r.y));
    asm("v_cvt_pk_bf16_f32 %0, %1, %2" : "=v"(l1) : "v"(r.z), "v"(r.w));
    if (off != 0xffffffffu) {
      *reinterpret_cast<u2x_t *>(smem + off) = u2x_t{h0, h1};
      *reinterpret_cast<u2x_t *>(smem + off + 64) = u2x_t{m0, m1};
      *reinterpret_cast<u2x_t *>(smem + off + 128) = u2x_t{l0, l1};
    }
  }
}
template <int NP>
__device__ __forceinline__ void split_mfma(f32x16 &acc, f32x16 &lo, const v4f &ah, const v4f &am, const v4f &al, const v4f &bh, const v4f &bm, const v4f &bl) {
  typedef __bf16 bf16x8 __attribute__((ext_vector_type(8)));
  typedef _Float16 f16x8 __attribute__((ext_vector_type(8)));
  if (NP == 2) {
    lo = __builtin_amdgcn_mfma_f32_32x32x16_f16(__builtin_bit_cast(f16x8, bm), __builtin_bit_cast(f16x8, ah), lo, 0, 0, 0);
    acc = __builtin_amdgcn_mfma_f32_32x32x16_f16(__builtin_bit_cast(f16x8, bh), __builtin_bit_cast(f16x8, ah), acc, 0, 0, 0);
    lo = __builtin_amdgcn_mfma_f32_32x32x16_f16(__builtin_bit_cast(f16x8, bh), __builtin_bit_cast(f16x8, am), lo, 0, 0, 0);
  } else {
    acc = __builtin_amdgcn_mfma_f32_32x32x16_bf16(__builtin_bit_cast(bf16x8, bm), __builtin_bit_cast(bf16x8, am), acc, 0, 0, 0);
    acc = __builtin_amdgcn_mfma_f32_32x32x16_bf16(__builtin_bit_cast(bf16x8, bh), __builtin_bit_cast(bf16x8, al), acc, 0, 0, 0);
    acc = __builtin_amdgcn_mfma_f32_32x32x16_bf16(__builtin_bit_cast(bf16x8, bl), __builtin_bit_cast(bf16x8, ah), acc, 0, 0, 0);
    acc = __builtin_amdgcn_mfma_f32_32x32x16_bf16(__builtin_bit_cast(bf16x8, bh), __builtin_bit_cast(bf16x8, am), acc, 0, 0, 0);
    acc = __builtin_amdgcn_mfma_f32_32x32x16_bf16(__builtin_bit_cast(bf16x8, bm), __builtin_bit_cast(bf16x8, ah), acc, 0, 0, 0);
    acc = __builtin_amdgcn_mfma_f32_32x32x16_bf16(__builtin_bit_cast(bf16x8, bh), __builtin_bit_cast(bf16x8, ah), acc, 0, 0, 0);
  }
}
template <int NP>
__device__ __forceinline__ void split_finish(f32x16 &acc, const f32x16 &lo, unsigned amax, int lane, int *status) {
  if (NP == 2) {
#pragma unroll
    for (int r = 0; r < 16; ++r) acc[r] = __builtin_fmaf(lo[r], 1.f / 2048.f, acc[r]);
    if (__builtin_amdgcn_ballot_w64(amax > F16_MAX_BITS) != 0 && lane == 0) atomicOr(status, STATUS_F16_SPLIT_RANGE);
  }
}

#ifndef MSI_S2X3_NSTG
#define MSI_S2X3_NSTG 2
#endif
template <int NP, int TH = 4>
struct HaloGeomS2X3 {
  static constexpr int PW = 17, PH = TH + 1, NPX = PW * PH;
  static constexpr int PIX_BYTES = NP * 64 + 16;
  static constexpr int ROW_PITCH = ((PW * PIX_BYTES + 127) / 256) * 256 + 128;
  static constexpr int A_BYTES = PH * ROW_PITCH;
  static constexpr int B_ROW = 64, B_PLANE = 64 * B_ROW, B_STAGE = NP * B_PLANE;
  static constexpr int NSTG = NP == 3 ? MSI_S2X3_NSTG : 3;
  static constexpr int LDS_BYTES = A_BYTES + NSTG * B_STAGE;
  static constexpr int NLOAD = (NPX * 8 + 255) / 256;
};

#ifndef MSI_S2X_WAVES
#define MSI_S2X_WAVES 3
#ifndef MSI_S2X3_ABLATE
#define MSI_S2X3_ABLATE 0
#endif
#endif
template <int APPLY, int NP, int TH>
__device__ __forceinline__ void conv_halo_s2_x3_body(const ConvParams &p, char *smem) {
  typedef HaloGeomS2X3<NP, TH> G;
  constexpr int PW = G::PW, NPX = G::NPX, NLOAD = G::NLOAD;
  constexpr int MT = TH / 4, NT = 1, BM = 16 * TH;
  static_assert(TH == 4 || (TH == 8 && NP == 3 && G::NSTG == 2), "the 8-row tile: six-product form, two-stage ring");
  const int tid = threadIdx.x, lane = tid & 63;
  const int wave = __builtin_amdgcn_readfirstlane(tid >> 6);
  const int wm = wave >> 1, wn = wave & 1;
  const int CH = p.cpt0;
  int t, c0 = 0, c1 = CH, ks = 0, slot = 0;
  {
    const int bid = blockIdx.x;
    if (bid < p.nb_main && p.split0 == 1) {
      const int q = p.n_main >> 3, r = p.n_main & 7, xcd = bid & 7, local = bid >> 3;
      t = (xcd < r ? xcd * (q + 1) : r * (q + 1) + (xcd - r) * q) + local;
    } else {
      int sp, r, tbase;
      unsigned mg;
      if (bid < p.nb_main) { sp = p.split0; mg = p.mg_sp0; r = bid; tbase = 0; }
      else { sp = p.split; mg = p.mg_sp; r = bid - p.nb_main; tbase = p.n_main; }
      const int tl = (int)udiv_magic((unsigned)r, (unsigned)sp, mg);
      ks = r - tl * sp;
      t = tbase + tl;
      c0 = (int)udiv_magic((unsigned)(ks * CH), (unsigned)sp, mg);
      c1 = (int)udiv_magic((unsigned)((ks + 1) * CH), (unsigned)sp, mg);
      slot = bid - (p.split0 == 1 ? p.nb_main : 0);
    }
  }
  const bool full = (c0 == 0) & (c1 == CH);
  int tile_m, tile_n, b;
  {
    int r = t;
    const int q1 = (int)udiv_magic((unsigned)r, (unsigned)p.tiles_m, p.mg_tm);
    tile_m = r - q1 * p.tiles_m; r = q1;
    const int q2 = (int)udiv_magic((unsigned)r, (unsigned)p.tiles_n, p.mg_tn);
    tile_n = r - q2 * p.tiles_n;
    b = q2;
  }
  const int tyi = (int)udiv_magic((unsigned)tile_m, (unsigned)p.halo_tx, p.mg_htx);
  const int oh0 = tyi * TH, ow0 = (tile_m - tyi * p.halo_tx) * 16;
  const int H = p.Hin, W = p.Win, C = p.C0;
  const int S = p.ksteps;
  const int plane_bytes = p.npad * G::B_ROW;
  const __amdgpu_buffer_rsrc_t rsrc_b = __builtin_amdgcn_make_buffer_rsrc((void *)p.wpk_x3, 0, (int)((size_t)S * NP * plane_bytes), 0x00020000);
  const unsigned b_voff = (unsigned)((tile_n * 64 + wave * 16 + (lane >> 2)) * G::B_ROW + (lane & 3) * 16);
  auto b_issue = [&](const int c, const int tap, const int st) __attribute__((always_inline)) {
    if (MSI_S2X3_ABLATE & 1) return;
    char *sB_ = smem + G::A_BYTES + st * G::B_STAGE + wave * 16 * G::B_ROW;
    const int soff_ = (tap * CH + c) * NP * plane_bytes;
    __builtin_amdgcn_raw_ptr_buffer_load_lds(rsrc_b, (lds_void *)sB_, 16, b_voff, soff_, 0, 0);
    __builtin_amdgcn_raw_ptr_buffer_load_lds(rsrc_b, (lds_void *)(sB_ + G::B_PLANE), 16, b_voff, soff_ + plane_bytes, 0, 0);
    if (NP == 3) __builtin_amdgcn_raw_ptr_buffer_load_lds(rsrc_b, (lds_void *)(sB_ + 2 * G::B_PLANE), 16, b_voff, soff_ + 2 * plane_bytes, 0, 0);
  };
  b_issue(c0, 0, 0);
  if (G::NSTG == 3) b_issue(c0, 2, 1);

  unsigned voff[4][NLOAD], lds_a[NLOAD];
  bool pok[4][NLOAD];
  const int cslot = tid & 7;
  const size_t in_bytes = (size_t)H * W * C * 4;
  const __amdgpu_buffer_rsrc_t rsrc_a = __builtin_amdgcn_make_buffer_rsrc((void *)(p.x0 + (size_t)b * in_bytes), 0, (int)in_bytes, 0x00020000);
  v4f araw[NLOAD], g4, be4;
  unsigned amax_ = 0u;
#pragma unroll
  for (int u = 0; u < 4; ++u) {
#pragma unroll
    for (int k = 0; k < NLOAD; ++k) {
      const int pp = (tid + 256 * k) >> 3;
      const int py = pp / PW, px = pp - py * PW;
      if (u == 0) lds_a[k] = pp < NPX ? (unsigned)(py * G::ROW_PITCH + px * G::PIX_BYTES + cslot * 8) : 0xffffffffu;
      const int ih = 2 * (oh0 + py) + (u >> 1) - p.pad_t;
      int iw = 2 * (ow0 + px) + (u & 1) - p.pad_l;
      if (p.wrap) iw = iw < 0 ? iw + W : (iw >= W ? iw - W : iw);
      pok[u][k] = pp < NPX && ih >= 0 && ih < H && iw >= 0 && iw < W;
      voff[u][k] = pok[u][k] ? __umul24((unsigned)(ih * W + iw), (unsigned)(C * 4)) + (unsigned)(cslot * 16) : OOB;
    }
    if (u == 0) {
#pragma unroll
      for (int k = 0; k < NLOAD; ++k)
        araw[k] = __builtin_bit_cast(v4f, (u32x4_t)__builtin_amdgcn_raw_buffer_load_b128(rsrc_a, voff[0][k], c0 * ROW_BYTES, 0));
      if (APPLY) {
        g4 = *reinterpret_cast<const v4f *>(p.ln_gamma + c0 * 32 + cslot * 4);
        be4 = *reinterpret_cast<const v4f *>(p.ln_beta + c0 * 32 + cslot * 4);
      }
      __builtin_amdgcn_sched_barrier(0);
    }
  }

  float inv_f = 1.f, mu_hi = 0.f, mu_lo = 0.f;
  bool has_pad = false;
  if (APPLY) {
    bool bad = false;
#pragma unroll
    for (int k = 0; k < NLOAD; ++k)
#pragma unroll
      for (int u = 0; u < 4; ++u) bad |= (lds_a[k] != 0xffffffffu) && !pok[u][k];
    has_pad = __builtin_amdgcn_ballot_w64(bad) != 0;
  }
  v4f s4 = {1.f, 1.f, 1.f, 1.f}, t4 = {0.f, 0.f, 0.f, 0.f};
  auto patch_load = [&](const int c, auto U_c) __attribute__((always_inline)) {
    constexpr int U = decltype(U_c)::value;
    if (MSI_S2X3_ABLATE & 64) return;
#pragma unroll
    for (int k_ = 0; k_ < NLOAD; ++k_)
      araw[k_] = __builtin_bit_cast(v4f, (u32x4_t)__builtin_amdgcn_raw_buffer_load_b128(rsrc_a, voff[U][k_], c * ROW_BYTES, 0));
    if (APPLY && U == 0) {
      g4 = *reinterpret_cast<const v4f *>(p.ln_gamma + c * 32 + cslot * 4);
      be4 = *reinterpret_cast<const v4f *>(p.ln_beta + c * 32 + cslot * 4);
    }
  };
  auto patch_store = [&](auto U_c) __attribute__((always_inline)) {
    constexpr int U = decltype(U_c)::value;
    if (APPLY && U == 0) {
      s4 = inv_f * g4;
      const v4f nh = {-mu_hi, -mu_hi, -mu_hi, -mu_hi}, nl = {-mu_lo, -mu_lo, -mu_lo, -mu_lo};
      t4 = __builtin_elementwise_fma(nl, s4, __builtin_elementwise_fma(nh, s4, be4));
    }
#pragma unroll
    for (int k_ = 0; k_ < NLOAD; ++k_) {
      v4f y = araw[k_];
      if (APPLY) {
        y = __builtin_elementwise_max(__builtin_elementwise_fma(y, s4, t4), v4f{0.f, 0.f, 0.f, 0.f});
        if (has_pad && !pok[U][k_]) y = v4f{0.f, 0.f, 0.f, 0.f};
      }
      split_store<NP>(smem, lds_a[k_], y, amax_);
    }
  };

  const int frow = lane & 31, fh = lane >> 5, fswz = (frow >> 1) & 7;
  const unsigned lds_base = (unsigned)(size_t)(lds_void *)smem;
  const unsigned a_base = lds_base + (unsigned)((2 * MT * wm + (frow >> 4)) * G::ROW_PITCH + ((frow & 15) ^ ((frow >> 4) << 3)) * G::PIX_BYTES + fh * 16);
  unsigned b_s[2];
  (void)fswz;
#pragma unroll
  for (int s_ = 0; s_ < 2; ++s_)
    b_s[s_] = lds_base + G::A_BYTES + (wn * 32 + frow) * G::B_ROW + (((2 * s_ + fh) ^ ((frow >> 2) & 3)) << 4);
  typedef __bf16 bf16x8 __attribute__((ext_vector_type(8), unused));
  f32x16 acc[MT][1], acc_lo;
#pragma unroll
  for (int r = 0; r < 16; ++r) {
    acc_lo[r] = 0.f;
#pragma unroll
    for (int i = 0; i < MT; ++i) acc[i][0][r] = 0.f;
  }

  int c = c0, cpar = 0;
  auto s2step = [&](auto J_c) __attribute__((always_inline)) {
    constexpr int J = decltype(J_c)::value;
    constexpr int TAP_ = s2_tap(J), U_ = s2_unit(J);
    constexpr int DY_ = (TAP_ / 3) >> 1, DX_ = (TAP_ % 3) >> 1;
    constexpr bool FIRST_ = J == 0 || J == 4 || J == 6 || J == 8, LAST_ = J == 3 || J == 5 || J == 7 || J == 8;
    constexpr int AOFF_ = DY_ * G::ROW_PITCH + DX_ * G::PIX_BYTES;
    const bool more_ = U_ < 3 || c + 1 < c1;
    const unsigned bst_ = (unsigned)(G::NSTG == 3 ? J % 3 : ((J ^ cpar) & 1)) * G::B_STAGE;
    if (G::NSTG == 2) {
      const int stn_ = ((J ^ cpar) & 1) ^ 1;
      if (J + 1 < 9) b_issue(c, s2_tap((J + 1) % 9), stn_);
      else if (c + 1 < c1) b_issue(c + 1, s2_tap(0), stn_);
    }
    v4f ah_[2], am_[2], al_[2], bh_[2], bm_[2], bl_[2];
    if constexpr (MT == 2) {
      constexpr int A1_ = AOFF_ + 2 * G::ROW_PITCH;
      v4f xh_[2][2], xm_[2][2], xl_[2][2];
      bh_[0] = lds_read128<0>(b_s[0] + bst_); bm_[0] = lds_read128<G::B_PLANE>(b_s[0] + bst_); bl_[0] = lds_read128<2 * G::B_PLANE>(b_s[0] + bst_);
      xh_[0][0] = lds_read128<AOFF_>(a_base); xm_[0][0] = lds_read128<AOFF_ + 64>(a_base); xl_[0][0] = lds_read128<AOFF_ + 128>(a_base);
      xh_[0][1] = lds_read128<A1_>(a_base); xm_[0][1] = lds_read128<A1_ + 64>(a_base); xl_[0][1] = lds_read128<A1_ + 128>(a_base);
      bh_[1] = lds_read128<0>(b_s[1] + bst_); bm_[1] = lds_read128<G::B_PLANE>(b_s[1] + bst_); bl_[1] = lds_read128<2 * G::B_PLANE>(b_s[1] + bst_);
      wait_lgkm6<6>(bh_[0], bm_[0], bl_[0], xh_[0][0], xm_[0][0], xl_[0][0]);
      split_mfma<3>(acc[0][0], acc_lo, xh_[0][0], xm_[0][0], xl_[0][0], bh_[0], bm_[0], bl_[0]);
      __builtin_amdgcn_sched_barrier(0);
      xh_[1][0] = lds_read128<AOFF_ + 32>(a_base); xm_[1][0] = lds_read128<AOFF_ + 96>(a_base); xl_[1][0] = lds_read128<AOFF_ + 160>(a_base);
      xh_[1][1] = lds_read128<A1_ + 32>(a_base); xm_[1][1] = lds_read128<A1_ + 96>(a_base); xl_[1][1] = lds_read128<A1_ + 160>(a_base);
      if (FIRST_ && more_) {
        if (U_ < 3) patch_load(c, IC<(U_ + 1) & 3>{});
        else patch_load(c + 1, IC<0>{});
      }
      wait_lgkm6<9>(xh_[0][1], xm_[0][1], xl_[0][1], bh_[0], bm_[0], bl_[0]);
      split_mfma<3>(acc[1][0], acc_lo, xh_[0][1], xm_[0][1], xl_[0][1], bh_[0], bm_[0], bl_[0]);
      __builtin_amdgcn_sched_barrier(0);
      wait_lgkm6<3>(bh_[1], bm_[1], bl_[1], xh_[1][0], xm_[1][0], xl_[1][0]);
      split_mfma<3>(acc[0][0], acc_lo, xh_[1][0], xm_[1][0], xl_[1][0], bh_[1], bm_[1], bl_[1]);
      __builtin_amdgcn_sched_barrier(0);
      wait_lgkm6<0>(xh_[1][1], xm_[1][1], xl_[1][1], bh_[1], bm_[1], bl_[1]);
      split_mfma<3>(acc[1][0], acc_lo, xh_[1][1], xm_[1][1], xl_[1][1], bh_[1], bm_[1], bl_[1]);
      __builtin_amdgcn_sched_barrier(0);
    } else {
    if (!(MSI_S2X3_ABLATE & 8))
#pragma unroll
    for (int s_ = 0; s_ < 2; ++s_) {
      ah_[s_] = s_ == 0 ? lds_read128<AOFF_>(a_base) : lds_read128<AOFF_ + 32>(a_base);
      bh_[s_] = lds_read128<0>(b_s[s_] + bst_);
      am_[s_] = s_ == 0 ? lds_read128<AOFF_ + 64>(a_base) : lds_read128<AOFF_ + 96>(a_base);
      bm_[s_] = lds_read128<G::B_PLANE>(b_s[s_] + bst_);
      if (NP == 3) {
        al_[s_] = s_ == 0 ? lds_read128<AOFF_ + 128>(a_base) : lds_read128<AOFF_ + 160>(a_base);
        bl_[s_] = lds_read128<2 * G::B_PLANE>(b_s[s_] + bst_);
      } else { al_[s_] = ah_[s_]; bl_[s_] = bh_[s_]; }
    }
#pragma unroll
    for (int s_ = 0; s_ < 2; ++s_) {
      if (NP == 3) {
        if (s_ == 0) wait_lgkm6<6>(ah_[0], bh_[0], am_[0], bm_[0], al_[0], bl_[0]);
        else wait_lgkm6<0>(ah_[1], bh_[1], am_[1], bm_[1], al_[1], bl_[1]);
      } else {
        if (s_ == 0) wait_lgkm4<4>(ah_[0], bh_[0], am_[0], bm_[0]);
        else wait_lgkm4<0>(ah_[1], bh_[1], am_[1], bm_[1]);
      }
      if (!(MSI_S2X3_ABLATE & 16)) split_mfma<NP>(acc[0][0], acc_lo, ah_[s_], am_[s_], al_[s_], bh_[s_], bm_[s_], bl_[s_]);
      __builtin_amdgcn_sched_barrier(0);
      if (s_ == 0) {
        if (FIRST_ && more_) {
          if (U_ < 3) patch_load(c, IC<(U_ + 1) & 3>{});
          else patch_load(c + 1, IC<0>{});
        }
        if (G::NSTG == 3) {
        if (J + 2 < 9) b_issue(c, s2_tap((J + 2) % 9), (J + 2) % 3);
        else if (c + 1 < c1) b_issue(c + 1, s2_tap((J + 2) % 9), (J + 2) % 3);
        }
      }
    }
    }
    {
      const bool issued_ = (J + 2 < 9) || (c + 1 < c1);
      if (G::NSTG == 2) {
        if (FIRST_ && !LAST_ && more_) wait_vmcnt<NLOAD>();
        else wait_vmcnt<0>();
      } else if (FIRST_ && !LAST_ && more_) wait_vmcnt<NP + NLOAD>();
      else if (issued_) wait_vmcnt<NP>();
      else wait_vmcnt<0>();
    }
    if (!(MSI_S2X3_ABLATE & 4)) __builtin_amdgcn_s_barrier();
    if (LAST_ && more_ && !(MSI_S2X3_ABLATE & 32)) {
      patch_store(IC<(U_ + 1) & 3>{});
      asm volatile("s_waitcnt lgkmcnt(0)" ::: "memory");
      __builtin_amdgcn_s_barrier();
    }
  };

  if (APPLY) {
    double *s_stat = reinterpret_cast<double *>(smem);
    ln_mean_inv(p.ln_sums + (size_t)b * LN_SHARDS * LN_WORDS, p.ln_inv_n, p.ln_scl_src, p.status, s_stat, tid);
    const double mu = s_stat[0];
    inv_f = (float)s_stat[1];
    mu_hi = (float)mu;
    mu_lo = (float)(mu - (double)mu_hi);
    __syncthreads();
  }
  wait_vmcnt<0>();
  patch_store(IC<0>{});
  asm volatile("s_waitcnt lgkmcnt(0)" ::: "memory");
  __builtin_amdgcn_s_barrier();
  for (; c < c1; ++c) {
    cpar = (c - c0) & 1;
    s2step(IC<0>{}); s2step(IC<1>{}); s2step(IC<2>{}); s2step(IC<3>{}); s2step(IC<4>{});
    s2step(IC<5>{}); s2step(IC<6>{}); s2step(IC<7>{}); s2step(IC<8>{});
  }
  split_finish<NP>(acc[0][0], acc_lo, amax_, lane, p.status);

  if (!full) {
    constexpr int SLAB = BM * 64 * 4;
    const __amdgpu_buffer_rsrc_t rsrc_p = __builtin_amdgcn_make_buffer_rsrc((void *)(p.partial + (size_t)slot * (BM * 64)), 0, SLAB, 0x00020000);
    if (p.tile_cnt == nullptr) {
      dump_acc<MT, NT, 0>(acc, rsrc_p, tid);
      return;
    }
    dump_acc<MT, NT, MSI_HANDOFF_AUX>(acc, rsrc_p, tid);
    const int nsp = t < p.n_main ? p.split0 : p.split;
    asm volatile("s_waitcnt vmcnt(0)" ::: "memory");
    handoff_release();
    __syncthreads();
    int *s_old = reinterpret_cast<int *>(smem);
    if (tid == 0)
      *s_old = __hip_atomic_fetch_add(p.tile_cnt + (t - (p.split0 == 1 ? p.n_main : 0)), 1, __ATOMIC_RELAXED, __HIP_MEMORY_SCOPE_AGENT);
    __syncthreads();
    if (*s_old != nsp - 1) return;
    handoff_acquire();
    const __amdgpu_buffer_rsrc_t rsrc_t = __builtin_amdgcn_make_buffer_rsrc((void *)(p.partial + (size_t)(slot - ks) * (BM * 64)), 0, nsp * SLAB, 0x00020000);
    sum_slabs<MT, NT, MSI_HANDOFF_AUX>(acc, rsrc_t, nsp, SLAB, tid);
    __syncthreads();
  }
  emit_tile<BM, 64, MODE_CONV>(p, acc, tile_m, tile_n, 0, b, tid, smem);
}

template <int APPLY, int NP>
__global__ void __launch_bounds__(256) __attribute__((amdgpu_waves_per_eu(NP == 2 ? MSI_S2X_WAVES : (MSI_S2X3_NSTG == 2 ? 3 : 2))))
conv_halo_s2_x3_kernel(const ConvParams p) {
#if defined(__HIP_DEVICE_COMPILE__)
  extern __shared__ __attribute__((aligned(16))) char smem[];
  conv_halo_s2_x3_body<APPLY, NP, 4>(p, smem);
#endif
}

template <int APPLY>
__global__ void __launch_bounds__(256) __attribute__((amdgpu_waves_per_eu(2)))
conv_halo8_s2_x3_kernel(const ConvParams p) {
#if defined(__HIP_DEVICE_COMPILE__)
  extern __shared__ __attribute__((aligned(16))) char smem[];
  conv_halo_s2_x3_body<APPLY, 3, 8>(p, smem);
#endif
}

template <int NS, int NPL, int TH = 4>
struct HaloGeomCT3 : HaloGeomX3<1, NS, NPL, TH> {
  typedef HaloGeomX3<1, NS, NPL, TH> B_;
  static constexpr int PH = TH + 1, NPX = B_::PW * PH;
  static constexpr int A_BYTES = PH * B_::ROW_PITCH;
  static constexpr int LDS_BYTES = A_BYTES + B_::NSTG * B_::B_STAGE;
  static constexpr int NLOAD = (NPX * 8 + 255) / 256;
};
#ifndef MSI_CT_MAXW
#define MSI_CT_MAXW 8
#endif
#ifndef MSI_CT3_ABLATE
#define MSI_CT3_ABLATE 0
#endif
#ifndef MSI_CT3_NSTG
#define MSI_CT3_NSTG 2
#endif
template <int NP, int TH>
__device__ __forceinline__ void convt_halo_x3_body(const ConvParams &p, char *smem) {
  typedef HaloGeomCT3<(NP == 3 ? MSI_CT3_NSTG : 3), NP, TH> G;
  constexpr int PW = G::PW, NPX = G::NPX, NLOAD = G::NLOAD, NSTG = G::NSTG, PD = NSTG - 1;
  constexpr int MT = TH / 4, BM = 16 * TH;
  static_assert(NSTG == 3 || NSTG == 2, "prefetch distance two or one");
  static_assert(TH == 4 || (TH == 8 && NP == 3 && NSTG == 2), "the 8-row tile: six-product form, two-stage ring");
  const int tid = threadIdx.x, lane = tid & 63;
  const int wave = __builtin_amdgcn_readfirstlane(tid >> 6);
  const int wm = wave >> 1, wn = wave & 1;
  const int CH = p.cpt0 + p.cpt1;
  int t, c0 = 0, c1 = CH, ks = 0, slot = 0;
  {
    const int bid = blockIdx.x;
    if (bid < p.nb_main && p.split0 == 1) {
      const int q = p.n_main >> 3, r = p.n_main & 7, xcd = bid & 7, local = bid >> 3;
      t = (xcd < r ? xcd * (q + 1) : r * (q + 1) + (xcd - r) * q) + local;
    } else {
      int sp, r, tbase;
      unsigned mg;
      if (bid < p.nb_main) { sp = p.split0; mg = p.mg_sp0; r = bid; tbase = 0; }
      else { sp = p.split; mg = p.mg_sp; r = bid - p.nb_main; tbase = p.n_main; }
      const int tl = (int)udiv_magic((unsigned)r, (unsigned)sp, mg);
      ks = r - tl * sp;
      t = tbase + tl;
      c0 = (int)udiv_magic((unsigned)(ks * CH), (unsigned)sp, mg);
      c1 = (int)udiv_magic((unsigned)((ks + 1) * CH), (unsigned)sp, mg);
      slot = bid - (p.split0 == 1 ? p.nb_main : 0);
    }
  }
  const bool full = (c0 == 0) & (c1 == CH);
  int ph, tile_m, tile_n, b;
  {
    int r = t;
    ph = r & 1; r >>= 1;
    const int q1 = (int)udiv_magic((unsigned)r, (unsigned)p.tiles_m, p.mg_tm);
    tile_m = r - q1 * p.tiles_m; r = q1;
    const int q2 = (int)udiv_magic((unsigned)r, (unsigned)p.tiles_n, p.mg_tn);
    tile_n = r - q2 * p.tiles_n;
    b = q2;
  }
  const int tyi = (int)udiv_magic((unsigned)tile_m, (unsigned)p.halo_tx, p.mg_htx);
  const int oh0 = tyi * TH, ow0 = (tile_m - tyi * p.halo_tx) * 16;
  const int H = p.Hin, W = p.Win;
  const int rowup = (ph && !p.wrap) ? 0 : 1;

  const int S = p.ksteps;
  const int plane_bytes = p.npad * G::B_ROW;
  const __amdgpu_buffer_rsrc_t rsrc_b = __builtin_amdgcn_make_buffer_rsrc((void *)p.wpk_x3, 0, (int)((size_t)4 * S * NP * plane_bytes), 0x00020000);
  const unsigned b_voff = (unsigned)((tile_n * 64 + wave * 16 + (lane >> 2)) * G::B_ROW + (lane & 3) * 16);
  auto b_issue = [&](const int cls, const int tap, const int c, const int st) __attribute__((always_inline)) {
    if (MSI_CT3_ABLATE & 1) return;
    char *sB_ = smem + G::A_BYTES + st * G::B_STAGE + wave * 16 * G::B_ROW;
    const int soff_ = (cls * S + tap * CH + c) * NP * plane_bytes;
    __builtin_amdgcn_raw_ptr_buffer_load_lds(rsrc_b, (lds_void *)sB_, 16, b_voff, soff_, 0, 0);
    __builtin_amdgcn_raw_ptr_buffer_load_lds(rsrc_b, (lds_void *)(sB_ + G::B_PLANE), 16, b_voff, soff_ + plane_bytes, 0, 0);
    if (NP == 3) __builtin_amdgcn_raw_ptr_buffer_load_lds(rsrc_b, (lds_void *)(sB_ + 2 * G::B_PLANE), 16, b_voff, soff_ + 2 * plane_bytes, 0, 0);
  };
  b_issue(2 * ph, 0, c0, 0);
  if (NSTG == 3) b_issue(2 * ph, 1, c0, 1);

  unsigned pixi[NLOAD], lds_a[NLOAD];
  bool pok[NLOAD];
  const int cslot = tid & 7;
#pragma unroll
  for (int k = 0; k < NLOAD; ++k) {
    const int pp = (tid + 256 * k) >> 3;
    const int py = pp / PW, px = pp - py * PW;
    const int ih = oh0 - rowup + py;
    int iw = ow0 - 1 + px;
    bool cok = iw >= 0 && iw < W;
    if (p.wrap) {
      cok = iw >= 0 && iw < W + 4;
      iw -= 2;
      iw = iw < 0 ? iw + W : (iw >= W ? iw - W : iw);
    }
    pok[k] = pp < NPX && ih >= 0 && ih < H && cok;
    pixi[k] = (unsigned)(ih * W + iw);
    lds_a[k] = pp < NPX ? (unsigned)(py * G::ROW_PITCH + px * G::PIX_BYTES + cslot * 8) : 0xffffffffu;
  }
  const size_t in0 = (size_t)H * W * p.C0 * 4, in1 = (size_t)H * W * p.C1 * 4;
  const __amdgpu_buffer_rsrc_t rsrc_a0 = __builtin_amdgcn_make_buffer_rsrc((void *)(p.x0 + (size_t)b * in0), 0, (int)in0, 0x00020000);
  const __amdgpu_buffer_rsrc_t rsrc_a1 = __builtin_amdgcn_make_buffer_rsrc((void *)(p.x1 + (size_t)b * in1), 0, (int)(in1 ? in1 : 16), 0x00020000);

  float inv_f[2] = {1.f, 1.f}, mu_hi[2] = {0.f, 0.f}, mu_lo[2] = {0.f, 0.f};
  bool has_pad = false;
  {
    bool bad = false;
#pragma unroll
    for (int k = 0; k < NLOAD; ++k) bad |= (lds_a[k] != 0xffffffffu) && !pok[k];
    has_pad = __builtin_amdgcn_ballot_w64(bad) != 0;
  }
  v4f araw[NLOAD], g4, be4;
  unsigned amax_ = 0u;
  int src_ld = 0;
  auto patch_load = [&](const int c) __attribute__((always_inline)) {
    if (MSI_CT3_ABLATE & 64) return;
    const int s_ = c >= p.cpt0 ? 1 : 0, cc_ = s_ ? c - p.cpt0 : c;
    const unsigned cb_ = (unsigned)((s_ ? p.C1 : p.C0) * 4);
    src_ld = s_;
    if (s_ == 0) {
#pragma unroll
      for (int k_ = 0; k_ < NLOAD; ++k_)
        araw[k_] = __builtin_bit_cast(v4f, (u32x4_t)__builtin_amdgcn_raw_buffer_load_b128(
            rsrc_a0, pok[k_] ? __umul24(pixi[k_], cb_) + (unsigned)(cslot * 16) : OOB, cc_ * ROW_BYTES, 0));
    } else {
#pragma unroll
      for (int k_ = 0; k_ < NLOAD; ++k_)
        araw[k_] = __builtin_bit_cast(v4f, (u32x4_t)__builtin_amdgcn_raw_buffer_load_b128(
            rsrc_a1, pok[k_] ? __umul24(pixi[k_], cb_) + (unsigned)(cslot * 16) : OOB, cc_ * ROW_BYTES, 0));
    }
    const float *gp_ = (s_ ? p.ln_gamma1 : p.ln_gamma), *bp_ = (s_ ? p.ln_beta1 : p.ln_beta);
    if ((p.halo_apply >> s_) & 1) {
      g4 = *reinterpret_cast<const v4f *>(gp_ + cc_ * 32 + cslot * 4);
      be4 = *reinterpret_cast<const v4f *>(bp_ + cc_ * 32 + cslot * 4);
    } else {
      g4 = *reinterpret_cast<const v4f *>(p.wpk + cslot * 16);
      be4 = *reinterpret_cast<const v4f *>(p.wpk + cslot * 16 + 128);
    }
  };
  auto patch_store = [&]() __attribute__((always_inline)) {
    const bool ap_ = (p.halo_apply >> src_ld) & 1;
    v4f s4 = {1.f, 1.f, 1.f, 1.f}, t4 = {0.f, 0.f, 0.f, 0.f};
    if (ap_) {
      const float ih_ = src_ld ? inv_f[1] : inv_f[0], mh_ = src_ld ? mu_hi[1] : mu_hi[0], ml_ = src_ld ? mu_lo[1] : mu_lo[0];
      s4 = ih_ * g4;
      const v4f nh = {-mh_, -mh_, -mh_, -mh_}, nl = {-ml_, -ml_, -ml_, -ml_};
      t4 = __builtin_elementwise_fma(nl, s4, __builtin_elementwise_fma(nh, s4, be4));
    }
#pragma unroll
    for (int k_ = 0; k_ < NLOAD; ++k_) {
      v4f y = araw[k_];
      if (ap_) {
        y = __builtin_elementwise_max(__builtin_elementwise_fma(y, s4, t4), v4f{0.f, 0.f, 0.f, 0.f});
        if (has_pad && !pok[k_]) y = v4f{0.f, 0.f, 0.f, 0.f};
      }
      split_store<NP>(smem, lds_a[k_], y, amax_);
    }
  };

  const int frow = lane & 31, fh = lane >> 5, fswz = (frow >> 1) & 7;
  const unsigned lds_base = (unsigned)(size_t)(lds_void *)smem;
  const unsigned a_base0 = lds_base + (unsigned)((rowup + 2 * MT * wm + (frow >> 4)) * G::ROW_PITCH + ((frow & 15) ^ ((frow >> 4) << 3)) * G::PIX_BYTES + fh * 16);
  const unsigned a_base1 = rowup ? a_base0 - G::ROW_PITCH : a_base0 + G::ROW_PITCH;
  const unsigned wadj = p.wrap ? 2u * G::PIX_BYTES : 0u;
  unsigned b_s[2];
  (void)fswz;
#pragma unroll
  for (int s_ = 0; s_ < 2; ++s_)
    b_s[s_] = lds_base + G::A_BYTES + (wn * 32 + frow) * G::B_ROW + (((2 * s_ + fh) ^ ((frow >> 2) & 3)) << 4);
  typedef __bf16 bf16x8 __attribute__((ext_vector_type(8), unused));
  f32x16 acc[2][MT][1], acc_lo[2];
#pragma unroll
  for (int cl = 0; cl < 2; ++cl)
#pragma unroll
    for (int r = 0; r < 16; ++r) {
      acc_lo[cl][r] = 0.f;
#pragma unroll
      for (int i = 0; i < MT; ++i) acc[cl][i][0][r] = 0.f;
    }

  int c = c0, st = 0;
  constexpr int NPLD = NLOAD + 2;
  auto ctstep = [&](auto J_c) __attribute__((always_inline)) {
    constexpr int J = decltype(J_c)::value;
    constexpr int PWC_ = J >> 2, TH_ = (J >> 1) & 1, TW_ = J & 1;
    constexpr int COFF_ = (1 + (PWC_ ? TW_ : -TW_)) * G::PIX_BYTES;
    const unsigned ab_ = (TH_ ? a_base1 : a_base0) - ((PWC_ && TW_) ? wadj : 0u);
    v4f ah_[2], am_[2], al_[2], bh_[2], bm_[2], bl_[2];
    const unsigned bst_ = (unsigned)st * G::B_STAGE;
    bool issued_ = false;
    if (NSTG == 2) {
      constexpr int JN_ = (J + 1) & 7;
      if (J + 1 < 8) { issued_ = true; b_issue(2 * ph + (JN_ >> 2), JN_ & 3, c, st ^ 1); }
      else if (c + 1 < c1) { issued_ = true; b_issue(2 * ph + (JN_ >> 2), JN_ & 3, c + 1, st ^ 1); }
    }
    if constexpr (MT == 2) {
      constexpr int C1_ = COFF_ + 2 * G::ROW_PITCH;
      v4f xh_[2][2], xm_[2][2], xl_[2][2];
      bh_[0] = lds_read128<0>(b_s[0] + bst_); bm_[0] = lds_read128<G::B_PLANE>(b_s[0] + bst_); bl_[0] = lds_read128<2 * G::B_PLANE>(b_s[0] + bst_);
      xh_[0][0] = lds_read128<COFF_>(ab_); xm_[0][0] = lds_read128<COFF_ + 64>(ab_); xl_[0][0] = lds_read128<COFF_ + 128>(ab_);
      xh_[0][1] = lds_read128<C1_>(ab_); xm_[0][1] = lds_read128<C1_ + 64>(ab_); xl_[0][1] = lds_read128<C1_ + 128>(ab_);
      bh_[1] = lds_read128<0>(b_s[1] + bst_); bm_[1] = lds_read128<G::B_PLANE>(b_s[1] + bst_); bl_[1] = lds_read128<2 * G::B_PLANE>(b_s[1] + bst_);
      wait_lgkm6<6>(bh_[0], bm_[0], bl_[0], xh_[0][0], xm_[0][0], xl_[0][0]);
      split_mfma<3>(acc[PWC_][0][0], acc_lo[PWC_], xh_[0][0], xm_[0][0], xl_[0][0], bh_[0], bm_[0], bl_[0]);
      __builtin_amdgcn_sched_barrier(0);
      xh_[1][0] = lds_read128<COFF_ + 32>(ab_); xm_[1][0] = lds_read128<COFF_ + 96>(ab_); xl_[1][0] = lds_read128<COFF_ + 160>(ab_);
      xh_[1][1] = lds_read128<C1_ + 32>(ab_); xm_[1][1] = lds_read128<C1_ + 96>(ab_); xl_[1][1] = lds_read128<C1_ + 160>(ab_);
      if (J == 0 && c + 1 < c1) patch_load(c + 1);
      wait_lgkm6<9>(xh_[0][1], xm_[0][1], xl_[0][1], bh_[0], bm_[0], bl_[0]);
      split_mfma<3>(acc[PWC_][1][0], acc_lo[PWC_], xh_[0][1], xm_[0][1], xl_[0][1], bh_[0], bm_[0], bl_[0]);
      __builtin_amdgcn_sched_barrier(0);
      wait_lgkm6<3>(bh_[1], bm_[1], bl_[1], xh_[1][0], xm_[1][0], xl_[1][0]);
      split_mfma<3>(acc[PWC_][0][0], acc_lo[PWC_], xh_[1][0], xm_[1][0], xl_[1][0], bh_[1], bm_[1], bl_[1]);
      __builtin_amdgcn_sched_barrier(0);
      wait_lgkm6<0>(xh_[1][1], xm_[1][1], xl_[1][1], bh_[1], bm_[1], bl_[1]);
      split_mfma<3>(acc[PWC_][1][0], acc_lo[PWC_], xh_[1][1], xm_[1][1], xl_[1][1], bh_[1], bm_[1], bl_[1]);
      __builtin_amdgcn_sched_barrier(0);
    } else {
    if (!(MSI_CT3_ABLATE & 8))
#pragma unroll
    for (int s_ = 0; s_ < 2; ++s_) {
      ah_[s_] = s_ == 0 ? lds_read128<COFF_>(ab_) : lds_read128<COFF_ + 32>(ab_);
      bh_[s_] = lds_read128<0>(b_s[s_] + bst_);
      am_[s_] = s_ == 0 ? lds_read128<COFF_ + 64>(ab_) : lds_read128<COFF_ + 96>(ab_);
      bm_[s_] = lds_read128<G::B_PLANE>(b_s[s_] + bst_);
      if (NP == 3) {
        al_[s_] = s_ == 0 ? lds_read128<COFF_ + 128>(ab_) : lds_read128<COFF_ + 160>(ab_);
        bl_[s_] = lds_read128<2 * G::B_PLANE>(b_s[s_] + bst_);
      } else { al_[s_] = ah_[s_]; bl_[s_] = bh_[s_]; }
    }
#pragma unroll
    for (int s_ = 0; s_ < 2; ++s_) {
      if (NP == 3) {
        if (s_ == 0) wait_lgkm6<6>(ah_[0], bh_[0], am_[0], bm_[0], al_[0], bl_[0]);
        else wait_lgkm6<0>(ah_[1], bh_[1], am_[1], bm_[1], al_[1], bl_[1]);
      } else {
        if (s_ == 0) wait_lgkm4<4>(ah_[0], bh_[0], am_[0], bm_[0]);
        else wait_lgkm4<0>(ah_[1], bh_[1], am_[1], bm_[1]);
      }
      if (!(MSI_CT3_ABLATE & 16)) split_mfma<NP>(acc[PWC_][0][0], acc_lo[PWC_], ah_[s_], am_[s_], al_[s_], bh_[s_], bm_[s_], bl_[s_]);
      __builtin_amdgcn_sched_barrier(0);
      if (s_ == 0) {
        if (J == 0 && c + 1 < c1) patch_load(c + 1);
        if (NSTG == 3) {
        int sn_ = st + PD; sn_ = sn_ >= NSTG ? sn_ - NSTG : sn_;
        constexpr int JN_ = (J + PD) & 7;
        if (J + PD < 8) { issued_ = true; b_issue(2 * ph + (JN_ >> 2), JN_ & 3, c, sn_); }
        else if (c + 1 < c1) { issued_ = true; b_issue(2 * ph + (JN_ >> 2), JN_ & 3, c + 1, sn_); }
        }
      }
    }
    }
    if (NSTG == 2) {
      if (J == 0 && c + 1 < c1) wait_vmcnt<NPLD>();
      else wait_vmcnt<0>();
    } else if (J == 0 && c + 1 < c1) wait_vmcnt<NP + NPLD>();
    else if (issued_) wait_vmcnt<NP>();
    else wait_vmcnt<0>();
    if (!(MSI_CT3_ABLATE & 4)) __builtin_amdgcn_s_barrier();
    st = st + 1 == NSTG ? 0 : st + 1;
  };

  patch_load(c0);
  if (p.halo_apply) {
    double *s_stat = reinterpret_cast<double *>(smem);
    if (p.halo_apply & 1) {
      ln_mean_inv(p.ln_sums + (size_t)b * LN_SHARDS * LN_WORDS, p.ln_inv_n, p.ln_scl_src, p.status, s_stat, tid);
      const double mu = s_stat[0];
      inv_f[0] = (float)s_stat[1]; mu_hi[0] = (float)mu; mu_lo[0] = (float)(mu - (double)mu_hi[0]);
      __syncthreads();
    }
    if (p.halo_apply & 2) {
      ln_mean_inv(p.ln_sums1 + (size_t)b * LN_SHARDS * LN_WORDS, p.ln_inv_n1, p.ln_scl_src1, p.status, s_stat, tid);
      const double mu = s_stat[0];
      inv_f[1] = (float)s_stat[1]; mu_hi[1] = (float)mu; mu_lo[1] = (float)(mu - (double)mu_hi[1]);
      __syncthreads();
    }
  }
  wait_vmcnt<0>();
  patch_store();
  asm volatile("s_waitcnt lgkmcnt(0)" ::: "memory");
  __builtin_amdgcn_s_barrier();
  for (; c < c1; ++c) {
    ctstep(IC<0>{}); ctstep(IC<1>{}); ctstep(IC<2>{}); ctstep(IC<3>{}); ctstep(IC<4>{}); ctstep(IC<5>{}); ctstep(IC<6>{}); ctstep(IC<7>{});
    if (c + 1 < c1 && !(MSI_CT3_ABLATE & 32)) {
      patch_store();
      asm volatile("s_waitcnt lgkmcnt(0)" ::: "memory");
      __builtin_amdgcn_s_barrier();
    }
  }
  split_finish<NP>(acc[0][0][0], acc_lo[0], amax_, lane, p.status);
  split_finish<NP>(acc[1][0][0], acc_lo[1], amax_, lane, p.status);

  if (!full) {
    constexpr int SLAB = BM * 64 * 4;
    if (p.tile_cnt == nullptr) {
#pragma unroll
      for (int cl = 0; cl < 2; ++cl) {
        const __amdgpu_buffer_rsrc_t rsrc_p = __builtin_amdgcn_make_buffer_rsrc((void *)(p.partial + ((size_t)slot * 2 + cl) * (BM * 64)), 0, SLAB, 0x00020000);
        dump_acc<MT, 1, 0>(acc[cl], rsrc_p, tid);
      }
      return;
    }
#pragma unroll
    for (int cl = 0; cl < 2; ++cl) {
      const __amdgpu_buffer_rsrc_t rsrc_p = __builtin_amdgcn_make_buffer_rsrc((void *)(p.partial + ((size_t)slot * 2 + cl) * (BM * 64)), 0, SLAB, 0x00020000);
      dump_acc<MT, 1, MSI_HANDOFF_AUX>(acc[cl], rsrc_p, tid);
    }
    const int nsp = t < p.n_main ? p.split0 : p.split;
    asm volatile("s_waitcnt vmcnt(0)" ::: "memory");
    handoff_release();
    __syncthreads();
    int *s_old = reinterpret_cast<int *>(smem);
    if (tid == 0)
      *s_old = __hip_atomic_fetch_add(p.tile_cnt + (t - (p.split0 == 1 ? p.n_main : 0)), 1, __ATOMIC_RELAXED, __HIP_MEMORY_SCOPE_AGENT);
    __syncthreads();
    if (*s_old != nsp - 1) return;
    handoff_acquire();
#pragma unroll
    for (int cl = 0; cl < 2; ++cl) {
      const __amdgpu_buffer_rsrc_t rsrc_t = __builtin_amdgcn_make_buffer_rsrc((void *)(p.partial + ((size_t)(slot - ks) * 2 + cl) * (BM * 64)), 0, nsp * 2 * SLAB, 0x00020000);
      sum_slabs<MT, 1, MSI_HANDOFF_AUX>(acc[cl], rsrc_t, nsp, 2 * SLAB, tid);
    }
  }
#pragma unroll
  for (int cl = 0; cl < 2; ++cl) emit_tile<BM, 64, MODE_CONVT>(p, acc[cl], tile_m, tile_n, 2 * ph + cl, b, tid);
}

template <int NP>
__global__ void __launch_bounds__(256) __attribute__((amdgpu_waves_per_eu(2, MSI_CT_MAXW)))
convt_halo_x3_kernel(const ConvParams p) {
#if defined(__HIP_DEVICE_COMPILE__)
  extern __shared__ __attribute__((aligned(16))) char smem[];
  convt_halo_x3_body<NP, 4>(p, smem);
#endif
}

__global__ void __launch_bounds__(256) __attribute__((amdgpu_waves_per_eu(2)))
convt_halo8_x3_kernel(const ConvParams p) {
#if defined(__HIP_DEVICE_COMPILE__)
  extern __shared__ __attribute__((aligned(16))) char smem[];
  convt_halo_x3_body<3, 8>(p, smem);
#endif
}

template <int R, int A, int N>
int launch_s1(const LayerLaunch &Q, const ConvParams &p, hipStream_t stream) {
  return launch_kernel<conv_halo_x3_kernel<R, A, N>, HaloGeomX3<R, x3_nstg(R, N), N>::LDS_BYTES>(Q.nblocks, p, stream, "conv_halo_x3");
}
template <int A, int N>
int launch_s2(const LayerLaunch &Q, const ConvParams &p, hipStream_t stream) {
  return launch_kernel<conv_halo_s2_x3_kernel<A, N>, HaloGeomS2X3<N>::LDS_BYTES>(Q.nblocks, p, stream, "conv_halo_x3");
}

}

namespace msi_cnn {
int launch_x3(const LayerLaunch &Q, const ConvParams &p, hipStream_t stream) {
  const ConvVariant &V = Q.variant;
  typedef HaloGeomX3<1, (MSI_X3_NSTG ? MSI_X3_NSTG : 2), 3, 8> G8;
  typedef HaloGeomS2X3<3, 8> G8s;
  switch (vkey(V.family, V.rate, V.apply, V.planes)) {
    case vkey(CONV_HALO_X3, 1, 0, 2): return launch_s1<1, 0, 2>(Q, p, stream);
    case vkey(CONV_HALO_X3, 1, 0, 3): return launch_s1<1, 0, 3>(Q, p, stream);
    case vkey(CONV_HALO_X3, 1, 1, 2): return launch_s1<1, 1, 2>(Q, p, stream);
    case vkey(CONV_HALO_X3, 1, 1, 3): return launch_s1<1, 1, 3>(Q, p, stream);
    case vkey(CONV_HALO_X3, 2, 0, 2): return launch_s1<2, 0, 2>(Q, p, stream);
    case vkey(CONV_HALO_X3, 2, 0, 3): return launch_s1<2, 0, 3>(Q, p, stream);
    case vkey(CONV_HALO_X3, 2, 1, 2): return launch_s1<2, 1, 2>(Q, p, stream);
    case vkey(CONV_HALO_X3, 2, 1, 3): return launch_s1<2, 1, 3>(Q, p, stream);
    case vkey(CONV_HALO_X3, 3, 0, 2): return launch_s1<3, 0, 2>(Q, p, stream);
    case vkey(CONV_HALO_X3, 3, 0, 3): return launch_s1<3, 0, 3>(Q, p, stream);
    case vkey(CONV_HALO_X3, 3, 1, 2): return launch_s1<3, 1, 2>(Q, p, stream);
    case vkey(CONV_HALO_X3, 3, 1, 3): return launch_s1<3, 1, 3>(Q, p, stream);
    case vkey(CONV_HALO8_X3, 0, 0, 3): return launch_kernel<conv_halo8_x3_kernel<0, 3>, G8::LDS_BYTES>(Q.nblocks, p, stream, "conv_halo_x3");
    case vkey(CONV_HALO8_X3, 0, 1, 3): return launch_kernel<conv_halo8_x3_kernel<1, 3>, G8::LDS_BYTES>(Q.nblocks, p, stream, "conv_halo_x3");
    case vkey(CONV_HALO_S2_X3, 0, 0, 2): return launch_s2<0, 2>(Q, p, stream);
    case vkey(CONV_HALO_S2_X3, 0, 0, 3): return launch_s2<0, 3>(Q, p, stream);
    case vkey(CONV_HALO_S2_X3, 0, 1, 2): return launch_s2<1, 2>(Q, p, stream);
    case vkey(CONV_HALO_S2_X3, 0, 1, 3): return launch_s2<1, 3>(Q, p, stream);
    case vkey(CONV_HALO8_S2_X3, 0, 0): return launch_kernel<conv_halo8_s2_x3_kernel<0>, G8s::LDS_BYTES>(Q.nblocks, p, stream, "conv_halo_x3");
    case vkey(CONV_HALO8_S2_X3, 0, 1): return launch_kernel<conv_halo8_s2_x3_kernel<1>, G8s::LDS_BYTES>(Q.nblocks, p, stream, "conv_halo_x3");
    case vkey(CONVT_HALO_X3, 0, 0, 2): return launch_kernel<convt_halo_x3_kernel<2>, HaloGeomCT3<3, 2>::LDS_BYTES>(Q.nblocks, p, stream, "convt_halo_x3");
    case vkey(CONVT_HALO_X3, 0, 0, 3): return launch_kernel<convt_halo_x3_kernel<3>, HaloGeomCT3<MSI_CT3_NSTG, 3>::LDS_BYTES>(Q.nblocks, p, stream, "convt_halo_x3");
    case vkey(CONVT_HALO8_X3): return launch_kernel<convt_halo8_x3_kernel, HaloGeomCT3<MSI_CT3_NSTG, 3, 8>::LDS_BYTES>(Q.nblocks, p, stream, "convt_halo_x3");
  }
  return msi::fail(MSI_E_UNSUPPORTED, "conv_halo_x3: no split kernel of family %d with rate %d, APPLY %d, %d planes", V.family, V.rate, V.apply, V.planes);
}
}
```

Baseline: 570.3.

## Hoist LN shard, scale and coord-bias loads ahead of x3 conv main loops

Moves loads of layer-norm shard sums, ln_scl scale factors and coord-bias vectors to kernel entry in the x3 conv and convT halo kernels, so their global-memory latency overlaps the main MFMA loop instead of stalling the prologue or epilogue. It extends coord-bias preloading to multi-row tiles (MT>1) and merges the two ln_mean_inv barriers in the convT kernel into one. It also adds optional timing stamps under MSI_CONV_TIMING. The cost is higher register pressure from carrying the preloaded values through the loop, which could lower occupancy.

```diff
diff --git a/matryodshka_amd/csrc/cnn_device.h b/matryodshka_amd/csrc/cnn_device.h
--- a/matryodshka_amd/csrc/cnn_device.h
+++ b/matryodshka_amd/csrc/cnn_device.h
@@ -293,7 +293,7 @@
   }
   return r;
 }
-template <bool PRE>
+template <bool PRE, bool SYNC = true>
 __device__ __forceinline__ void ln_mean_inv_impl(const long long *sums, LnShard pre, double inv_n, const double *scl, int *status, double *s_stat, int tid) {
   static_assert(LN_SHARDS == 64, "one shard per lane of wave 0");
   const double inv_s1 = scl[2], inv_s2 = scl[3];
@@ -319,13 +319,16 @@
       s_stat[1] = r;
     }
   }
-  __syncthreads();
+  if constexpr (SYNC) __syncthreads();
 }
 __device__ __forceinline__ void ln_mean_inv(const long long *sums, double inv_n, const double *scl, int *status, double *s_stat, int tid) {
   ln_mean_inv_impl<false>(sums, LnShard{0, 0}, inv_n, scl, status, s_stat, tid);
 }
 __device__ __forceinline__ void ln_mean_inv_pre(LnShard pre, double inv_n, const double *scl, int *status, double *s_stat, int tid) {
   ln_mean_inv_impl<true>(nullptr, pre, inv_n, scl, status, s_stat, tid);
+}
+__device__ __forceinline__ void ln_mean_inv_pre_nosync(LnShard pre, double inv_n, const double *scl, int *status, double *s_stat, int tid) {
+  ln_mean_inv_impl<true, false>(nullptr, pre, inv_n, scl, status, s_stat, tid);
 }
 
 typedef unsigned u32x4_t __attribute__((ext_vector_type(4)));
@@ -400,7 +403,7 @@
 #endif
 template <int BM, int BN, int MODE, int RAW16, bool CB, bool STAGED, int WR>
 __device__ __forceinline__ void emit_whole_tile(const ConvParams &p, f32x16 (&acc)[BM / (32 * WR)][BN / 64], int tile_m, int tile_n, int cls,
-                                                int b, int tid, const v4f (&cb_pre)[4], bool use_pre, float pivot, float raw_mul,
+                                                int b, int tid, const v4f (&cb_pre)[4 * (BM / (32 * WR))], bool use_pre, float pivot, float raw_mul,
                                                 double scl_s1, double scl_s2, char *stage) {
   constexpr int MT = BM / (32 * WR), NT = BN / 64, NG = NT * 4, YSZ = RAW16 ? 2 : 4;
   constexpr int ROWB = NT * 32 * YSZ, PITCH = ROWB + 16, NP = ROWB / 16, PPI = 64 / NP, NRD = 32 / PPI;
@@ -458,7 +461,7 @@
       v4f cb[NG];
 #pragma unroll
       for (int q = 0; q < NG; ++q)
-        cb[q] = (MT == 1 && NT == 1 && use_pre) ? cb_pre[q & 3] : *reinterpret_cast<const v4f *>(cbp[i] + (q >> 2) * 32 + 8 * (q & 3));
+        cb[q] = (NT == 1 && use_pre) ? cb_pre[4 * i + (q & 3)] : *reinterpret_cast<const v4f *>(cbp[i] + (q >> 2) * 32 + 8 * (q & 3));
 #pragma unroll
       for (int q = 0; q < NG; ++q) { ya[q] += v2f{cb[q].x, cb[q].y}; yc[q] += v2f{cb[q].z, cb[q].w}; }
     }
@@ -541,8 +544,8 @@
 
 template <int BM, int BN, int MODE, bool INTERIOR, int RAW16, int WR>
 __device__ __forceinline__ void emit_tile_impl(const ConvParams &p, f32x16 (&acc)[BM / (32 * WR)][BN / 64], int tile_m,
-                                               int tile_n, int cls, int b, int tid, const v4f (&cb_pre)[4], bool use_pre, char *stage,
-                                               float raw_mul_pre) {
+                                               int tile_n, int cls, int b, int tid, const v4f (&cb_pre)[4 * (BM / (32 * WR))], bool use_pre, char *stage,
+                                               float raw_mul_pre, bool have_scl, double scl_s1_pre, double scl_s2_pre) {
   constexpr int MT = BM / (32 * WR), NT = BN / 64;
   const int lane = tid & 63, wave = tid >> 6, wm = wave >> 1, wn = wave & 1, half = lane >> 5;
   const int ph = cls >> 1, pw = cls & 1;
@@ -554,7 +557,8 @@
   const float pivot = __builtin_bit_cast(float, __builtin_amdgcn_readfirstlane(__builtin_bit_cast(int, acc[0][0][0])));
   double scl_s1 = 0.0, scl_s2 = 0.0;
   const bool have_pre = INTERIOR && RAW16 && MODE != MODE_HEAD && raw_mul_pre > 0.f;
-  if ((want_stats || RAW16) && !have_pre) { scl_s1 = p.ln_scl[0]; scl_s2 = p.ln_scl[1]; }
+  if ((want_stats || RAW16) && !have_pre && !have_scl) { scl_s1 = p.ln_scl[0]; scl_s2 = p.ln_scl[1]; }
+  if (have_scl) { scl_s1 = scl_s1_pre; scl_s2 = scl_s2_pre; }
   const float raw_mul = have_pre ? raw_mul_pre : RAW16 ? (float)(scl_s1 * (1.0 / 16777216.0)) : 1.f;
   constexpr int YSZ = RAW16 ? 2 : 4;
   float s1 = 0.f, s2 = 0.f, cnt = 0.f;
@@ -612,7 +616,7 @@
         v4f v = {acc[i][j][4 * g], acc[i][j][4 * g + 1], acc[i][j][4 * g + 2], acc[i][j][4 * g + 3]};
         if (ok) {
           if (has_cb) {
-            const v4f cb = (MT == 1 && NT == 1 && use_pre) ? cb_pre[g] : *reinterpret_cast<const v4f *>(cbrow + n);
+            const v4f cb = (NT == 1 && use_pre) ? cb_pre[4 * i + g] : *reinterpret_cast<const v4f *>(cbrow + n);
             v.x += cb.x; v.y += cb.y; v.z += cb.z; v.w += cb.w;
           }
           if (MODE == MODE_HEAD) {
@@ -677,18 +681,19 @@
 
 template <int BM, int BN, int MODE, int RAW16 = 0, int WR = 2>
 __device__ __forceinline__ void emit_tile(const ConvParams &p, f32x16 (&acc)[BM / (32 * WR)][BN / 64], int tile_m, int tile_n,
-                                          int cls, int b, int tid, const v4f (&cb_pre)[4], bool use_pre, char *stage = nullptr,
-                                          float raw_mul_pre = 0.f) {
+                                          int cls, int b, int tid, const v4f (&cb_pre)[4 * (BM / (32 * WR))], bool use_pre, char *stage = nullptr,
+                                          float raw_mul_pre = 0.f, bool have_scl = false, double scl_s1_pre = 0.0, double scl_s2_pre = 0.0) {
   const bool interior = !(MODE == MODE_CONVT && p.wrap != 0) && (tile_m + 1) * BM <= p.Mh * p.Mw &&
                         (tile_n + 1) * BN <= p.Cout && (p.Cout & 3) == 0;
-  if (interior) emit_tile_impl<BM, BN, MODE, true, RAW16, WR>(p, acc, tile_m, tile_n, cls, b, tid, cb_pre, use_pre, stage, raw_mul_pre);
-  else emit_tile_impl<BM, BN, MODE, false, RAW16, WR>(p, acc, tile_m, tile_n, cls, b, tid, cb_pre, use_pre, nullptr, 0.f);
+  if (interior) emit_tile_impl<BM, BN, MODE, true, RAW16, WR>(p, acc, tile_m, tile_n, cls, b, tid, cb_pre, use_pre, stage, raw_mul_pre, have_scl, scl_s1_pre, scl_s2_pre);
+  else emit_tile_impl<BM, BN, MODE, false, RAW16, WR>(p, acc, tile_m, tile_n, cls, b, tid, cb_pre, use_pre, nullptr, 0.f, have_scl, scl_s1_pre, scl_s2_pre);
 }
 template <int BM, int BN, int MODE, int RAW16 = 0, int WR = 2>
 __device__ __forceinline__ void emit_tile(const ConvParams &p, f32x16 (&acc)[BM / (32 * WR)][BN / 64], int tile_m, int tile_n,
-                                          int cls, int b, int tid, char *stage = nullptr, float raw_mul_pre = 0.f) {
-  const v4f none[4] = {};
-  emit_tile<BM, BN, MODE, RAW16, WR>(p, acc, tile_m, tile_n, cls, b, tid, none, false, stage, raw_mul_pre);
+                                          int cls, int b, int tid, char *stage = nullptr, float raw_mul_pre = 0.f,
+                                          bool have_scl = false, double scl_s1_pre = 0.0, double scl_s2_pre = 0.0) {
+  const v4f none[4 * (BM / (32 * WR))] = {};
+  emit_tile<BM, BN, MODE, RAW16, WR>(p, acc, tile_m, tile_n, cls, b, tid, none, false, stage, raw_mul_pre, have_scl, scl_s1_pre, scl_s2_pre);
 }
 
 __device__ __forceinline__ void load_coord_bias(const ConvParams &p, int tile_m, int tile_n, int tid, v4f (&cbv)[4]) {
@@ -709,6 +714,31 @@
   for (int g = 0; g < 4; ++g) {
     const int n = min(tile_n * 64 + wn * 32 + 4 * half + 8 * g, p.cb_stride - 4);
     cbv[g] = *reinterpret_cast<const v4f *>(cbrow + n);
+  }
+}
+template <int MT>
+__device__ __forceinline__ void load_coord_bias_mt(const ConvParams &p, int tile_m, int tile_n, int tid, v4f (&cbv)[4 * MT]) {
+  if constexpr (MT == 1) { load_coord_bias(p, tile_m, tile_n, tid, cbv); return; }
+#pragma unroll
+  for (int g = 0; g < 4 * MT; ++g) cbv[g] = v4f{0.f, 0.f, 0.f, 0.f};
+  if (p.coord_bias == nullptr) return;
+  const int lane = tid & 63, wave = tid >> 6, wm = wave >> 1, wn = wave & 1, half = lane >> 5;
+#pragma unroll
+  for (int i = 0; i < MT; ++i) {
+    const int local = wm * (MT * 32) + i * 32 + (lane & 31);
+    int m = tile_m * (64 * MT) + local;
+    if (p.halo_tx) {
+      const int tyi = (int)udiv_magic((unsigned)tile_m, (unsigned)p.halo_tx, p.mg_htx);
+      m = halo_row(p, tyi, local >> 4, 4 * MT) * p.Mw + (tile_m - tyi * p.halo_tx) * 16 + ((local & 15) ^ (((local >> 4) & 1) * p.halo_xor));
+    }
+    m = min(m, p.Mh * p.Mw - 1);
+    const int mh = (int)udiv_magic((unsigned)m, (unsigned)p.Mw, p.mg_mw), mw = m - mh * p.Mw;
+    const float *cbrow = p.coord_bias + (size_t)(mh * COORD_CLASSES + coord_class(mw, p.Mw)) * p.cb_stride;
+#pragma unroll
+    for (int g = 0; g < 4; ++g) {
+      const int n = min(tile_n * 64 + wn * 32 + 4 * half + 8 * g, p.cb_stride - 4);
+      cbv[4 * i + g] = *reinterpret_cast<const v4f *>(cbrow + n);
+    }
   }
 }
 
diff --git a/matryodshka_amd/csrc/cnn_igemm.hip b/matryodshka_amd/csrc/cnn_igemm.hip
--- a/matryodshka_amd/csrc/cnn_igemm.hip
+++ b/matryodshka_amd/csrc/cnn_igemm.hip
@@ -62,7 +62,7 @@
     b = q2;
   }
   constexpr bool CB_PRE = BM == 64 && BN == 64 && MODE == MODE_CONV && !BF16;
-  v4f cbv[4];
+  v4f cbv[4 * (BM / 64)];
   if constexpr (CB_PRE) load_coord_bias(p, tile_m, tile_n, tid, cbv);
   const int ph = cls >> 1, pw = cls & 1;
   const int mtot = p.Mh * p.Mw;
diff --git a/matryodshka_amd/csrc/cnn_x3.hip b/matryodshka_amd/csrc/cnn_x3.hip
--- a/matryodshka_amd/csrc/cnn_x3.hip
+++ b/matryodshka_amd/csrc/cnn_x3.hip
@@ -51,6 +51,18 @@
 #endif
 #ifndef MSI_X2_LATE_CB
 #define MSI_X2_LATE_CB 1
+#endif
+#ifndef MSI_X3_EARLY_LN
+#define MSI_X3_EARLY_LN 1
+#endif
+#ifndef MSI_X3_CB8
+#define MSI_X3_CB8 1
+#endif
+#ifndef MSI_S2X3_EARLY_CB
+#define MSI_S2X3_EARLY_CB 1
+#endif
+#ifndef MSI_X3_EARLY_SCL
+#define MSI_X3_EARLY_SCL 1
 #endif
 template <int NP>
 __device__ __forceinline__ void split_mfma(f32x16 &acc, f32x16 &lo, const v4f &ah, const v4f &am, const v4f &al, const v4f &bh, const v4f &bm, const v4f &bl);
@@ -102,8 +114,11 @@
   const int tyi = (int)udiv_magic((unsigned)tile_m, (unsigned)p.halo_tx, p.mg_htx);
   const int ow0 = (tile_m - tyi * p.halo_tx) * 16;
   const int H = p.Hin, W = p.Win, C = p.C0;
-  v4f cbv[4] = {};
-  if (MT == 1 && (!MSI_X2_LATE_CB || NPL != 2)) load_coord_bias(p, tile_m, tile_n, tid, cbv);
+  const bool have_scl = MSI_X3_EARLY_SCL && p.ln_scl != nullptr;
+  const double scl_s1 = have_scl ? p.ln_scl[0] : 0.0, scl_s2 = have_scl ? p.ln_scl[1] : 0.0;
+  v4f cbv[4 * MT] = {};
+  constexpr bool CB_EARLY = (MT == 1 || MSI_X3_CB8) && (!MSI_X2_LATE_CB || NPL != 2);
+  if (CB_EARLY) load_coord_bias_mt<MT>(p, tile_m, tile_n, tid, cbv);
   const int S = p.ksteps;
   const int plane_bytes = p.npad * G::B_ROW;
   const __amdgpu_buffer_rsrc_t rsrc_b = __builtin_amdgcn_make_buffer_rsrc((void *)p.wpk_x3, 0, (int)((size_t)S * NPL * plane_bytes), 0x00020000);
@@ -348,7 +363,7 @@
       __builtin_amdgcn_s_barrier();
     }
   }
-  if (MSI_X2_LATE_CB && NPL == 2) load_coord_bias(p, tile_m, tile_n, tid, cbv);
+  if (MSI_X2_LATE_CB && NPL == 2) load_coord_bias_mt<MT>(p, tile_m, tile_n, tid, cbv);
   if (NPL == 2) {
 #pragma unroll
     for (int r = 0; r < 16; ++r) acc[0][0][r] = __builtin_fmaf(acc_lo[r], 1.f / 2048.f, acc[0][0][r]);
@@ -391,7 +406,7 @@
     sum_slabs<MT, NT, MSI_HANDOFF_AUX>(acc, rsrc_t, nsp, SLAB, tid);
     __syncthreads();
   }
-  emit_tile<BM, 64, MODE_CONV>(p, acc, tile_m, tile_n, 0, b, tid, cbv, MT == 1 && p.coord_bias != nullptr, smem);
+  emit_tile<BM, 64, MODE_CONV>(p, acc, tile_m, tile_n, 0, b, tid, cbv, (MT == 1 || MSI_X3_CB8) && p.coord_bias != nullptr, smem, 0.f, have_scl, scl_s1, scl_s2);
 #ifdef MSI_CONV_TIMING
   stamp();
 #endif
@@ -499,6 +514,9 @@
   constexpr int PW = G::PW, NPX = G::NPX, NLOAD = G::NLOAD;
   constexpr int MT = TH / 4, NT = 1, BM = 16 * TH;
   static_assert(TH == 4 || (TH == 8 && NP == 3 && G::NSTG == 2), "the 8-row tile: six-product form, two-stage ring");
+#ifdef MSI_CONV_TIMING
+  const unsigned long long ts0 = __builtin_amdgcn_s_memtime(), ts0r = __builtin_amdgcn_s_memrealtime();
+#endif
   const int tid = threadIdx.x, lane = tid & 63;
   const int wave = __builtin_amdgcn_readfirstlane(tid >> 6);
   const int wm = wave >> 1, wn = wave & 1;
@@ -532,6 +550,13 @@
     tile_n = r - q2 * p.tiles_n;
     b = q2;
   }
+  LnShard shard = {0, 0};
+  if (APPLY && MSI_X3_EARLY_LN) shard = ln_shard_load(p.ln_sums + (size_t)b * LN_SHARDS * LN_WORDS, tid);
+  const bool have_scl = MSI_X3_EARLY_SCL && p.ln_scl != nullptr;
+  const double scl_s1 = have_scl ? p.ln_scl[0] : 0.0, scl_s2 = have_scl ? p.ln_scl[1] : 0.0;
+  constexpr bool CB_EARLY = MSI_S2X3_EARLY_CB == 1 && (TH == 8 || NP == 3), CB_LATE = MSI_S2X3_EARLY_CB != 0 && !CB_EARLY;
+  v4f cbv[4 * MT] = {};
+  if (CB_EARLY) load_coord_bias_mt<MT>(p, tile_m, tile_n, tid, cbv);
   const int tyi = (int)udiv_magic((unsigned)tile_m, (unsigned)p.halo_tx, p.mg_htx);
   const int oh0 = tyi * TH, ow0 = (tile_m - tyi * p.halo_tx) * 16;
   const int H = p.Hin, W = p.Win, C = p.C0;
@@ -734,7 +759,8 @@
 
   if (APPLY) {
     double *s_stat = reinterpret_cast<double *>(smem);
-    ln_mean_inv(p.ln_sums + (size_t)b * LN_SHARDS * LN_WORDS, p.ln_inv_n, p.ln_scl_src, p.status, s_stat, tid);
+    if (MSI_X3_EARLY_LN) ln_mean_inv_pre(shard, p.ln_inv_n, p.ln_scl_src, p.status, s_stat, tid);
+    else ln_mean_inv(p.ln_sums + (size_t)b * LN_SHARDS * LN_WORDS, p.ln_inv_n, p.ln_scl_src, p.status, s_stat, tid);
     const double mu = s_stat[0];
     inv_f = (float)s_stat[1];
     mu_hi = (float)mu;
@@ -745,18 +771,36 @@
   patch_store(IC<0>{});
   asm volatile("s_waitcnt lgkmcnt(0)" ::: "memory");
   __builtin_amdgcn_s_barrier();
+#ifdef MSI_CONV_TIMING
+  const unsigned long long ts1 = __builtin_amdgcn_s_memtime();
+#endif
   for (; c < c1; ++c) {
     cpar = (c - c0) & 1;
     s2step(IC<0>{}); s2step(IC<1>{}); s2step(IC<2>{}); s2step(IC<3>{}); s2step(IC<4>{});
     s2step(IC<5>{}); s2step(IC<6>{}); s2step(IC<7>{}); s2step(IC<8>{});
   }
+  if (CB_LATE) load_coord_bias_mt<MT>(p, tile_m, tile_n, tid, cbv);
   split_finish<NP>(acc[0][0], acc_lo, amax_, lane, p.status);
 
+#ifdef MSI_CONV_TIMING
+  const unsigned long long ts2 = __builtin_amdgcn_s_memtime();
+  auto stamp = [&]() __attribute__((always_inline)) {
+    if (p.dbg && tid == 0) {
+      unsigned long long *o = p.dbg + (size_t)blockIdx.x * 24;
+      o[0] = ts0; o[1] = ts1; o[2] = ts2; o[3] = __builtin_amdgcn_s_memtime(); o[22] = ts0r; o[23] = __builtin_amdgcn_s_memrealtime();
+      o[4] = __builtin_amdgcn_s_getreg(4 | (31 << 11));
+      o[5] = __builtin_amdgcn_s_getreg(20 | (31 << 11));
+    }
+  };
+#endif
   if (!full) {
     constexpr int SLAB = BM * 64 * 4;
     const __amdgpu_buffer_rsrc_t rsrc_p = __builtin_amdgcn_make_buffer_rsrc((void *)(p.partial + (size_t)slot * (BM * 64)), 0, SLAB, 0x00020000);
     if (p.tile_cnt == nullptr) {
       dump_acc<MT, NT, 0>(acc, rsrc_p, tid);
+#ifdef MSI_CONV_TIMING
+      stamp();
+#endif
       return;
     }
     dump_acc<MT, NT, MSI_HANDOFF_AUX>(acc, rsrc_p, tid);
@@ -774,7 +818,10 @@
     sum_slabs<MT, NT, MSI_HANDOFF_AUX>(acc, rsrc_t, nsp, SLAB, tid);
     __syncthreads();
   }
-  emit_tile<BM, 64, MODE_CONV>(p, acc, tile_m, tile_n, 0, b, tid, smem);
+  emit_tile<BM, 64, MODE_CONV>(p, acc, tile_m, tile_n, 0, b, tid, cbv, (CB_EARLY || CB_LATE) && p.coord_bias != nullptr, smem, 0.f, have_scl, scl_s1, scl_s2);
+#ifdef MSI_CONV_TIMING
+  stamp();
+#endif
 }
 
 template <int APPLY, int NP>
@@ -819,6 +866,9 @@
   constexpr int MT = TH / 4, BM = 16 * TH;
   static_assert(NSTG == 3 || NSTG == 2, "prefetch distance two or one");
   static_assert(TH == 4 || (TH == 8 && NP == 3 && NSTG == 2), "the 8-row tile: six-product form, two-stage ring");
+#ifdef MSI_CONV_TIMING
+  const unsigned long long ts0 = __builtin_amdgcn_s_memtime(), ts0r = __builtin_amdgcn_s_memrealtime();
+#endif
   const int tid = threadIdx.x, lane = tid & 63;
   const int wave = __builtin_amdgcn_readfirstlane(tid >> 6);
   const int wm = wave >> 1, wn = wave & 1;
@@ -853,6 +903,13 @@
     tile_n = r - q2 * p.tiles_n;
     b = q2;
   }
+  LnShard shard0 = {0, 0}, shard1 = {0, 0};
+  if (MSI_X3_EARLY_LN) {
+    if (p.halo_apply & 1) shard0 = ln_shard_load(p.ln_sums + (size_t)b * LN_SHARDS * LN_WORDS, tid);
+    if (p.halo_apply & 2) shard1 = ln_shard_load(p.ln_sums1 + (size_t)b * LN_SHARDS * LN_WORDS, tid);
+  }
+  const bool have_scl = MSI_X3_EARLY_SCL && p.ln_scl != nullptr;
+  const double scl_s1 = have_scl ? p.ln_scl[0] : 0.0, scl_s2 = have_scl ? p.ln_scl[1] : 0.0;
   const int tyi = (int)udiv_magic((unsigned)tile_m, (unsigned)p.halo_tx, p.mg_htx);
   const int oh0 = tyi * TH, ow0 = (tile_m - tyi * p.halo_tx) * 16;
   const int H = p.Hin, W = p.Win;
@@ -1056,7 +1113,21 @@
   };
 
   patch_load(c0);
-  if (p.halo_apply) {
+  if (MSI_X3_EARLY_LN && p.halo_apply) {
+    double *s_stat = reinterpret_cast<double *>(smem);
+    if (p.halo_apply & 1) ln_mean_inv_pre_nosync(shard0, p.ln_inv_n, p.ln_scl_src, p.status, s_stat, tid);
+    if (p.halo_apply & 2) ln_mean_inv_pre_nosync(shard1, p.ln_inv_n1, p.ln_scl_src1, p.status, s_stat + 2, tid);
+    __syncthreads();
+    if (p.halo_apply & 1) {
+      const double mu = s_stat[0];
+      inv_f[0] = (float)s_stat[1]; mu_hi[0] = (float)mu; mu_lo[0] = (float)(mu - (double)mu_hi[0]);
+    }
+    if (p.halo_apply & 2) {
+      const double mu = s_stat[2];
+      inv_f[1] = (float)s_stat[3]; mu_hi[1] = (float)mu; mu_lo[1] = (float)(mu - (double)mu_hi[1]);
+    }
+    __syncthreads();
+  } else if (p.halo_apply) {
     double *s_stat = reinterpret_cast<double *>(smem);
     if (p.halo_apply & 1) {
       ln_mean_inv(p.ln_sums + (size_t)b * LN_SHARDS * LN_WORDS, p.ln_inv_n, p.ln_scl_src, p.status, s_stat, tid);
@@ -1075,6 +1146,9 @@
   patch_store();
   asm volatile("s_waitcnt lgkmcnt(0)" ::: "memory");
   __builtin_amdgcn_s_barrier();
+#ifdef MSI_CONV_TIMING
+  const unsigned long long ts1 = __builtin_amdgcn_s_memtime();
+#endif
   for (; c < c1; ++c) {
     ctstep(IC<0>{}); ctstep(IC<1>{}); ctstep(IC<2>{}); ctstep(IC<3>{}); ctstep(IC<4>{}); ctstep(IC<5>{}); ctstep(IC<6>{}); ctstep(IC<7>{});
     if (c + 1 < c1 && !(MSI_CT3_ABLATE & 32)) {
@@ -1086,6 +1160,17 @@
   split_finish<NP>(acc[0][0][0], acc_lo[0], amax_, lane, p.status);
   split_finish<NP>(acc[1][0][0], acc_lo[1], amax_, lane, p.status);
 
+#ifdef MSI_CONV_TIMING
+  const unsigned long long ts2 = __builtin_amdgcn_s_memtime();
+  auto stamp = [&]() __attribute__((always_inline)) {
+    if (p.dbg && tid == 0) {
+      unsigned long long *o = p.dbg + (size_t)blockIdx.x * 24;
+      o[0] = ts0; o[1] = ts1; o[2] = ts2; o[3] = __builtin_amdgcn_s_memtime(); o[22] = ts0r; o[23] = __builtin_amdgcn_s_memrealtime();
+      o[4] = __builtin_amdgcn_s_getreg(4 | (31 << 11));
+      o[5] = __builtin_amdgcn_s_getreg(20 | (31 << 11));
+    }
+  };
+#endif
   if (!full) {
     constexpr int SLAB = BM * 64 * 4;
     if (p.tile_cnt == nullptr) {
@@ -1094,6 +1179,9 @@
         const __amdgpu_buffer_rsrc_t rsrc_p = __builtin_amdgcn_make_buffer_rsrc((void *)(p.partial + ((size_t)slot * 2 + cl) * (BM * 64)), 0, SLAB, 0x00020000);
         dump_acc<MT, 1, 0>(acc[cl], rsrc_p, tid);
       }
+#ifdef MSI_CONV_TIMING
+      stamp();
+#endif
       return;
     }
 #pragma unroll
@@ -1118,7 +1206,10 @@
     }
   }
 #pragma unroll
-  for (int cl = 0; cl < 2; ++cl) emit_tile<BM, 64, MODE_CONVT>(p, acc[cl], tile_m, tile_n, 2 * ph + cl, b, tid);
+  for (int cl = 0; cl < 2; ++cl) emit_tile<BM, 64, MODE_CONVT>(p, acc[cl], tile_m, tile_n, 2 * ph + cl, b, tid, nullptr, 0.f, have_scl, scl_s1, scl_s2);
+#ifdef MSI_CONV_TIMING
+  stamp();
+#endif
 }
 
 template <int NP>
```

Result: no change. 568.9 (-0.2%).
